# VITA-Group/SinNeRF

Hardware: AMD Instinct MI355X
Metric: rendered rays/sec (64+64 samples), lego 400x400 (higher is better)
Workload: dtype f32; 1 GPU; nerf_synthetic/lego-shaped 400x400 frame (160000 rays/GPU), N_samples=64, N_importance=64, eval render (perturb=0, noise_std=0, white_back), random-init teacher weights; points_per_ray=192, parallelism=rays sharded x1, no collective

## Files before the change

include/sinnerf_hip.h:

```cpp
#ifndef SINNERF_HIP_H
#define SINNERF_HIP_H
#include <stdint.h>
#ifdef __cplusplus
extern "C" {
#endif

#define SN_ABI_VERSION 5

#define SN_DTYPE_F32 0
#define SN_DTYPE_BF16 1
#define SN_DTYPE_BF16_STATE 2
#define SN_DTYPE_BF16X3 3
#define SN_DTYPE_F16 4
#define SN_DTYPE_CLASSIC_HEADS 0x100
#define SN_DTYPE_COMPILER_SCHEDULED 0x200
#define SN_DTYPE_EMB_BF16 0x400

#define SN_E_BADARG (-1)
#define SN_E_TOOLARGE (-2)
#define SN_E_MISSING_RNG (-3)
#define SN_E_UNSUPPORTED (-4)
#define SN_E_BADSHAPE (-5)

#define SN_FLAG_BF16_COMPILER_SCHEDULED 2
#define SN_FLAG_F32_LDS_RING 4

int sn_abi_version(void);
const char* sn_error_string(int code);

int sn_layout_xyz_slot_col(int lane_half, int slot);
int sn_layout_dir_slot_col(int lane_half, int slot);
int sn_layout_slab_k(int slab);
int sn_layout_n_slabs(void);

#define SN_N_RAW_TENSORS 24
long sn_packed_weights_bytes(int dtype);
long sn_pack_table_entries(void);
long sn_pack_table_entries_dtype(int dtype);
int sn_build_pack_table(int dtype, int32_t* table_host);
int sn_pack_weights(const float* const* raw_host_array_of_device_ptrs, const int32_t* table, long n_entries,
                    void* blob, int dtype, void* stream);
long sn_packed_weights_bytes_bwd(void);
long sn_pack_table_entries_bwd(void);
int sn_build_pack_table_bwd(int32_t* table_host);
long sn_packed_weights_bytes_bwd_bf16(void);
long sn_pack_table_entries_bwd_bf16(void);
int sn_build_pack_table_bwd_bf16(int32_t* table_host);
long sn_packed_weights_bytes_bwd_bf16x3(void);
long sn_pack_table_entries_bwd_bf16x3(void);
int sn_build_pack_table_bwd_bf16x3(int32_t* table_host);

int sn_sample_coarse(const float* rays, long n_rays, int n_samples, int use_disp, float perturb,
                     const float* perturb_rand, float* z_vals, void* stream);

int sn_mlp_forward(const void* blob, int dtype, const float* rays, const float* z_vals, long n_rays, int n_samples,
                   int sigma_only, int flags, float* out, void* stream);

int sn_mlp_forward_train(const void* blob, int dtype, const float* rays, const float* z_vals, long n_rays, int n_samples,
                         float* out, float* acts, float* emb, long slot_rows, void* stream);

int sn_mlp_forward_train_embedded(const void* blob, int dtype, const float* x, long n_rows, int ld, float* out,
                                  float* acts, long slot_rows, void* stream);

int sn_mlp_backward_chain(const void* blob_bwd, int dtype, const float* acts, const float* out_raw, const float* g_raw,
                          long n_points, long slot_rows, float* g_acts, float* g_out, void* stream);

int sn_dw_gemm(const void* tasks, int n_tasks, void* stream);

long sn_weight_grads_workspace_bytes(long slot_rows, int dtype);
int sn_weight_grads(const void* acts, const float* emb, const void* g_acts, long slot_rows, int dtype, void* workspace,
                    float* const* grads_host_array_of_device_ptrs, int accumulate, void* stream);

int sn_composite_backward(const float* raw, const float* z_vals, const float* rays, const float* noise, float noise_std,
                          long n_rays, int n_samples, int white_back, const float* g_rgb, const float* g_depth,
                          const float* g_weights, float* g_raw, void* stream);

int sn_mlp_forward_embedded(const void* blob, int dtype, const float* x, long n_rows, int ld, int sigma_only,
                            int flags, float* out, void* stream);

int sn_composite_forward(const float* raw, int has_rgb, const float* z_vals, const float* rays, const float* noise,
                         float noise_std, long n_rays, int n_samples, int white_back, float* rgb, float* depth,
                         float* weights, void* stream);

int sn_sample_pdf(const float* z_vals, const float* weights, const float* u, long n_rays, int n_samples,
                  int n_importance, float* z_fine, float* z_merged, void* stream);

int sn_sample_pdf_bins(const float* bins, const float* weights, const float* u, long n_rays, int n_bins,
                       int n_importance, float eps, float* samples, void* stream);


int sn_generate_rays(const float* c2w, int H, int W, float focal, float near, float far, int x0, int y0, int stride_x,
                     int stride_y, int patch_w, int patch_h, float* rays, void* stream);

int sn_adam_step(float* params, const float* grads, float* exp_avg, float* exp_avg_sq, long n, float lr, float beta1,
                 float beta2, float eps, float weight_decay, int step, void* stream);

long sn_render_loss_workspace_bytes(void);
int sn_render_loss(const float* rgb_coarse, const float* rgb_fine, const float* depth_coarse, const float* depth_fine,
                   const float* rgb_gt, const float* depth_gt, const unsigned char* mask, int mask_mode, long n,
                   float w_rgb, float w_depth, float* g_rgb_coarse, float* g_rgb_fine, float* g_depth_coarse,
                   float* g_depth_fine, void* workspace, float* out, void* stream);

#ifdef __cplusplus
}
#endif
#endif
```

sinnerf_amd/_lib.py:

```python
import ctypes
import os

_HERE = os.path.dirname(os.path.abspath(__file__))
LIB_PATH = os.environ.get("SINNERF_HIP_LIB") or os.path.join(_HERE, "csrc", "libsinnerf_hip.so")

SN_DTYPE_F32 = 0
SN_DTYPE_BF16 = 1
SN_DTYPE_BF16_STATE = 2
SN_DTYPE_BF16X3 = 3
SN_DTYPE_F16 = 4
SN_DTYPE_CLASSIC_HEADS = 0x100
SN_FLAG_F32_LDS_RING = 4
SN_DTYPE_COMPILER_SCHEDULED = 0x200
N_RAW_TENSORS = 24
SN_DTYPE_EMB_BF16 = 0x400
ABI_VERSION = 5

c_fp = ctypes.c_void_p
c_vp = ctypes.c_void_p
_long, _int, _float = ctypes.c_long, ctypes.c_int, ctypes.c_float

SIGNATURES = {
    "sn_abi_version": (_int, []),
    "sn_error_string": (ctypes.c_char_p, [_int]),
    "sn_layout_xyz_slot_col": (_int, [_int, _int]),
    "sn_layout_dir_slot_col": (_int, [_int, _int]),
    "sn_layout_slab_k": (_int, [_int]),
    "sn_layout_n_slabs": (_int, []),
    "sn_packed_weights_bytes": (_long, [_int]),
    "sn_pack_table_entries": (_long, []),
    "sn_pack_table_entries_dtype": (_long, [_int]),
    "sn_build_pack_table": (_int, [_int, c_vp]),
    "sn_pack_weights": (_int, [ctypes.POINTER(c_vp), c_vp, _long, c_vp, _int, c_vp]),
    "sn_packed_weights_bytes_bwd": (_long, []),
    "sn_pack_table_entries_bwd": (_long, []),
    "sn_build_pack_table_bwd": (_int, [c_vp]),
    "sn_packed_weights_bytes_bwd_bf16": (_long, []),
    "sn_pack_table_entries_bwd_bf16": (_long, []),
    "sn_build_pack_table_bwd_bf16": (_int, [c_vp]),
    "sn_packed_weights_bytes_bwd_bf16x3": (_long, []),
    "sn_pack_table_entries_bwd_bf16x3": (_long, []),
    "sn_build_pack_table_bwd_bf16x3": (_int, [c_vp]),
    "sn_sample_coarse": (_int, [c_fp, _long, _int, _int, _float, c_fp, c_fp, c_vp]),
    "sn_mlp_forward": (_int, [c_vp, _int, c_fp, c_fp, _long, _int, _int, _int, c_fp, c_vp]),
    "sn_mlp_forward_train": (_int, [c_vp, _int, c_fp, c_fp, _long, _int, c_fp, c_fp, c_fp, _long, c_vp]),
    "sn_mlp_forward_train_embedded": (_int, [c_vp, _int, c_fp, _long, _int, c_fp, c_fp, _long, c_vp]),
    "sn_mlp_backward_chain": (_int, [c_vp, _int, c_fp, c_fp, c_fp, _long, _long, c_fp, c_fp, c_vp]),
    "sn_dw_gemm": (_int, [c_vp, _int, c_vp]),
    "sn_weight_grads_workspace_bytes": (_long, [_long, _int]),
    "sn_weight_grads": (_int, [c_vp, c_fp, c_vp, _long, _int, c_vp, ctypes.POINTER(c_vp), _int, c_vp]),
    "sn_generate_rays": (_int, [c_fp, _int, _int, _float, _float, _float, _int, _int, _int, _int, _int, _int, c_fp, c_vp]),
    "sn_adam_step": (_int, [c_fp, c_fp, c_fp, c_fp, _long, _float, _float, _float, _float, _float, _int, c_vp]),
    "sn_render_loss_workspace_bytes": (_long, []),
    "sn_render_loss": (_int, [c_fp, c_fp, c_fp, c_fp, c_fp, c_fp, c_vp, _int, _long, _float, _float, c_fp, c_fp, c_fp, c_fp,
                              c_vp, c_fp, c_vp]),
    "sn_composite_backward": (_int, [c_fp, c_fp, c_fp, c_fp, _float, _long, _int, _int, c_fp, c_fp, c_fp, c_fp, c_vp]),
    "sn_mlp_forward_embedded": (_int, [c_vp, _int, c_fp, _long, _int, _int, _int, c_fp, c_vp]),
    "sn_composite_forward": (_int, [c_fp, _int, c_fp, c_fp, c_fp, _float, _long, _int, _int, c_fp, c_fp, c_fp, c_vp]),
    "sn_sample_pdf": (_int, [c_fp, c_fp, c_fp, _long, _int, _int, c_fp, c_fp, c_vp]),
    "sn_sample_pdf_bins": (_int, [c_fp, c_fp, c_fp, _long, _int, _int, _float, c_fp, c_vp]),
}


class SinnerfHipError(RuntimeError):
    pass


def _load():
    if not os.path.exists(LIB_PATH):
        raise ImportError(
            f"{LIB_PATH} not found: the HIP extension is not built. Run `python -c 'import __graft_entry__ as g; "
            "g.build()'` (or `make -C sinnerf_amd/csrc`). There is no CPU fallback for this path.")
    lib = ctypes.CDLL(LIB_PATH)
    for name, (res, args) in SIGNATURES.items():
        fn = getattr(lib, name)
        fn.restype, fn.argtypes = res, args
    if lib.sn_abi_version() != ABI_VERSION:
        raise ImportError(f"{LIB_PATH}: ABI version {lib.sn_abi_version()} != {ABI_VERSION}; rebuild the extension")
    return lib


lib = _load()


def check(code, what):
    if code != 0:
        msg = lib.sn_error_string(int(code))
        raise SinnerfHipError(f"{what} failed: [{code}] {msg.decode() if msg else '?'}")


def ptr(t):
    if t is None:
        return None
    assert t.is_contiguous(), "sinnerf_amd kernels need contiguous tensors"
    return ctypes.c_void_p(t.data_ptr())


def stream_ptr():
    import torch
    return ctypes.c_void_p(torch.cuda.current_stream().cuda_stream)
```

sinnerf_amd/autograd.py:

```python
import torch

from . import _lib
from .nerf import dtype_code


COMPILER_SCHEDULED = bool(int(__import__("os").environ.get("SINNERF_COMPILER_SCHEDULED", "0")))
EMB_BF16 = not bool(int(__import__("os").environ.get("SINNERF_EMB_FP32", "0")))


_EMB16_OK = None


def _emb16_supported():
    global _EMB16_OK
    if _EMB16_OK is None:
        _EMB16_OK = _lib.lib.sn_weight_grads_workspace_bytes(256, _lib.SN_DTYPE_BF16_STATE | _lib.SN_DTYPE_EMB_BF16) >= 0
    return _EMB16_OK


def _sched_flag():
    return _lib.SN_DTYPE_COMPILER_SCHEDULED if COMPILER_SCHEDULED else 0


def _state_code(model, acts, emb=None):
    if dtype_code(model.compute_dtype) == _lib.SN_DTYPE_BF16X3:
        return _lib.SN_DTYPE_BF16X3
    if dtype_code(model.compute_dtype) != _lib.SN_DTYPE_BF16:
        return _lib.SN_DTYPE_F32
    code = _lib.SN_DTYPE_BF16_STATE if acts.dtype == torch.bfloat16 else _lib.SN_DTYPE_BF16
    if emb is not None and emb.dtype == torch.bfloat16:
        code |= _lib.SN_DTYPE_EMB_BF16
    return code


def _sink_of(model, raws, needs):
    sink = getattr(model, "_grad_sink", None)
    if sink is None:
        return None
    for t, s_, need in zip(raws, sink, needs):
        if need and (t.grad is None or t.grad.data_ptr() != s_.data_ptr() or t.grad.shape != t.shape):
            return None
    return sink


def _weight_grads(model, acts, emb, G, needs):
    import ctypes
    dev = acts.device
    code = _state_code(model, acts, emb)
    rows = acts.shape[1]
    nbytes = _lib.lib.sn_weight_grads_workspace_bytes(rows, code)
    if nbytes < 0:
        _lib.check(int(nbytes), "sn_weight_grads_workspace_bytes")
    ws = torch.empty(int(nbytes), dtype=torch.uint8, device=dev)
    raws = model.raw_tensors()
    sink = _sink_of(model, raws, needs)
    if sink is not None:
        outs, accumulate = [s_ if need else None for s_, need in zip(sink, needs)], 1
    else:
        flat = torch.empty(sum(t.numel() for t, need in zip(raws, needs) if need), dtype=torch.float32, device=dev)
        outs, off, accumulate = [], 0, 0
        for t, need in zip(raws, needs):
            if need:
                outs.append(flat[off:off + t.numel()].view(t.shape))
                off += t.numel()
            else:
                outs.append(None)
    arr = (ctypes.c_void_p * _lib.N_RAW_TENSORS)(*[None if o is None else o.data_ptr() for o in outs])
    _lib.check(_lib.lib.sn_weight_grads(_lib.ptr(acts), _lib.ptr(emb), _lib.ptr(G), rows, code, _lib.ptr(ws), arr, accumulate,
                                        _lib.stream_ptr()), "sn_weight_grads")
    return [None] * len(outs) if sink is not None else outs


class _MLPFn(torch.autograd.Function):

    @staticmethod
    def forward(ctx, model, rays, z_vals, *params):
        embedded = z_vals is None
        n, s = (rays.shape[0], 1) if embedded else z_vals.shape
        P = n * s
        dev = rays.device
        code = dtype_code(model.compute_dtype)
        bf16 = code == _lib.SN_DTYPE_BF16
        if bf16:
            code = _lib.SN_DTYPE_BF16_STATE
        out = torch.empty((n, 4) if embedded else (n, s, 4), dtype=torch.float32, device=dev)
        tile = 256 if bf16 else 128
        rows = -(-P // tile) * tile
        acts = torch.empty((10, rows, 256), dtype=torch.bfloat16 if bf16 else torch.float32, device=dev)
        if embedded:
            emb = torch.zeros((rows, 128), dtype=torch.float32, device=dev)
            emb[:n, :63] = rays[:, :63]
            emb[:n, 64:91] = rays[:, 63:90]
            _lib.check(_lib.lib.sn_mlp_forward_train_embedded(_lib.ptr(model.packed()), model.kernel_dtype(code), _lib.ptr(rays), n, rays.shape[1],
                                                              _lib.ptr(out), _lib.ptr(acts), rows, _lib.stream_ptr()),
                       "sn_mlp_forward_train_embedded")
        else:
            emb16 = bf16 and EMB_BF16 and not COMPILER_SCHEDULED and P < 2 ** 31 - 256 and _emb16_supported()
            emb = torch.empty((rows, 128), dtype=torch.bfloat16 if emb16 else torch.float32, device=dev)
            flags = _sched_flag() | (_lib.SN_DTYPE_EMB_BF16 if emb16 else 0)
            _lib.check(_lib.lib.sn_mlp_forward_train(_lib.ptr(model.packed()), model.kernel_dtype(code) | flags, _lib.ptr(rays), _lib.ptr(z_vals), n, s,
                                                     _lib.ptr(out), _lib.ptr(acts), _lib.ptr(emb), rows, _lib.stream_ptr()),
                       "sn_mlp_forward_train")
        ctx.model = model
        ctx.n_points = P
        ctx.save_for_backward(acts, emb, out)
        return out

    @staticmethod
    def backward(ctx, g_out):
        acts, emb, out = ctx.saved_tensors
        model = ctx.model
        P, rows = ctx.n_points, acts.shape[1]
        dev = acts.device
        g_out = g_out.contiguous().float()
        G = torch.empty((10, rows, 256), dtype=acts.dtype, device=dev)
        if rows > P:
            G[:, P:].zero_()
        g_o = torch.empty((P, 4), dtype=torch.float32, device=dev)
        with torch.cuda.device(dev):
            code = dtype_code(model.compute_dtype)
            if acts.dtype == torch.bfloat16:
                code = _lib.SN_DTYPE_BF16_STATE
            _lib.check(_lib.lib.sn_mlp_backward_chain(_lib.ptr(model.packed_bwd(model.compute_dtype)), model.kernel_dtype(code) | _sched_flag(),
                                                      _lib.ptr(acts), _lib.ptr(out), _lib.ptr(g_out), P, rows, _lib.ptr(G),
                                                      _lib.ptr(g_o), _lib.stream_ptr()), "sn_mlp_backward_chain")
            needs = ctx.needs_input_grad[3:]
            grads = _weight_grads(model, acts, emb, G, needs)
        return (None, None, None, *grads)


class _CompositeFn(torch.autograd.Function):
    @staticmethod
    def forward(ctx, raw, z_vals, rays, noise, noise_std, white_back):
        n, s = z_vals.shape
        dev = rays.device
        ctx.set_materialize_grads(False)
        weights = torch.empty((n, s), dtype=torch.float32, device=dev)
        rgb = torch.empty((n, 3), dtype=torch.float32, device=dev)
        depth = torch.empty((n,), dtype=torch.float32, device=dev)
        _lib.check(_lib.lib.sn_composite_forward(_lib.ptr(raw), 1, _lib.ptr(z_vals), _lib.ptr(rays), _lib.ptr(noise),
                                                 float(noise_std), n, s, int(bool(white_back)), _lib.ptr(rgb),
                                                 _lib.ptr(depth), _lib.ptr(weights), _lib.stream_ptr()),
                   "sn_composite_forward")
        ctx.save_for_backward(raw, z_vals, rays, noise if noise is not None else torch.empty(0, device=dev))
        ctx.has_noise = noise is not None
        ctx.noise_std, ctx.white_back = float(noise_std), int(bool(white_back))
        return rgb, depth, weights

    @staticmethod
    def backward(ctx, g_rgb, g_depth, g_w):
        raw, z_vals, rays, noise = ctx.saved_tensors
        n, s = z_vals.shape
        g_raw = torch.empty((n, s, 4), dtype=torch.float32, device=raw.device)
        c = lambda t: None if t is None else t.contiguous().float()
        g_rgb, g_depth, g_w = c(g_rgb), c(g_depth), c(g_w)
        with torch.cuda.device(raw.device):
            _lib.check(_lib.lib.sn_composite_backward(_lib.ptr(raw), _lib.ptr(z_vals), _lib.ptr(rays),
                                                      _lib.ptr(noise) if ctx.has_noise else None, ctx.noise_std, n, s,
                                                      ctx.white_back, _lib.ptr(g_rgb), _lib.ptr(g_depth), _lib.ptr(g_w),
                                                      _lib.ptr(g_raw), _lib.stream_ptr()), "sn_composite_backward")
        return g_raw, None, None, None, None, None


def render_rays_autograd(models, rays, N_samples, use_disp, perturb, noise_std, N_importance, white_back, test_time,
                         detach_coarse):
    from . import rendering as R
    dev = rays.device
    n = rays.shape[0]
    stream = _lib.stream_ptr()
    for m in models:
        if dtype_code(m.compute_dtype) == _lib.SN_DTYPE_F16:
            raise NotImplementedError("sinnerf_amd: compute_dtype='fp16' is an INFERENCE arithmetic (sn_mlp_forward only); train in 'bf16' "
                                      "(same matrix rate), 'bf16x3' or 'fp32', or render under torch.no_grad()")
    perturb_rand = torch.rand((n, N_samples), device=dev) if perturb > 0 else None
    z_vals = torch.empty((n, N_samples), dtype=torch.float32, device=dev)
    _lib.check(_lib.lib.sn_sample_coarse(_lib.ptr(rays), n, N_samples, int(bool(use_disp)), float(perturb),
                                         _lib.ptr(perturb_rand), _lib.ptr(z_vals), stream), "sn_sample_coarse")
    result = {}
    coarse_grad = (not detach_coarse) and (not test_time) and any(p.requires_grad for p in models[0].parameters())
    if test_time:
        with torch.no_grad():
            raw_c = R._mlp(models[0], rays, z_vals, sigma_only=True)
    elif coarse_grad:
        raw_c = _MLPFn.apply(models[0], rays, z_vals, *models[0].raw_tensors())
    else:
        with torch.no_grad():
            raw_c = R._mlp(models[0], rays, z_vals, sigma_only=False)
    noise_c = torch.randn((n, N_samples), device=dev)
    noise_c = noise_c if noise_std != 0 else None
    if test_time:
        with torch.no_grad():
            _, _, w_c = R._composite(raw_c, False, z_vals, rays, noise_c, noise_std, white_back)
        result["opacity_coarse"] = w_c
    else:
        if coarse_grad:
            rgb_c, depth_c, w_c = _CompositeFn.apply(raw_c, z_vals, rays, noise_c, noise_std, white_back)
        else:
            with torch.no_grad():
                rgb_c, depth_c, w_c = R._composite(raw_c, True, z_vals, rays, noise_c, noise_std, white_back)
        result.update(rgb_coarse=rgb_c, depth_coarse=depth_c, opacity_coarse=w_c)
    if N_importance > 0:
        u = torch.rand((n, N_importance), device=dev) if perturb > 0 else None
        z_all = torch.empty((n, N_samples + N_importance), dtype=torch.float32, device=dev)
        _lib.check(_lib.lib.sn_sample_pdf(_lib.ptr(z_vals), _lib.ptr(w_c.detach()), _lib.ptr(u), n, N_samples,
                                          N_importance, None, _lib.ptr(z_all), stream), "sn_sample_pdf")
        if any(p.requires_grad for p in models[1].parameters()):
            raw_f = _MLPFn.apply(models[1], rays, z_all, *models[1].raw_tensors())
        else:
            with torch.no_grad():
                raw_f = R._mlp(models[1], rays, z_all, sigma_only=False)
        noise_f = torch.randn((n, N_samples + N_importance), device=dev)
        noise_f = noise_f if noise_std != 0 else None
        if raw_f.requires_grad:
            rgb_f, depth_f, w_f = _CompositeFn.apply(raw_f, z_all, rays, noise_f, noise_std, white_back)
        else:
            with torch.no_grad():
                rgb_f, depth_f, w_f = R._composite(raw_f, True, z_all, rays, noise_f, noise_std, white_back)
        result.update(rgb_fine=rgb_f, depth_fine=depth_f, opacity_fine=w_f)
    else:
        if test_time:
            raise NameError("name 'rgb_coarse' is not defined (render_rays(test_time=True) needs N_importance > 0, "
                            "as in the reference: rendering.py:331)")
        result.update(rgb_fine=result["rgb_coarse"], depth_fine=result["depth_coarse"],
                      opacity_fine=result["opacity_coarse"])
    return result


def mlp_embedded_autograd(model, x, sigma_only):
    if dtype_code(model.compute_dtype) == _lib.SN_DTYPE_F16:
        raise NotImplementedError("sinnerf_amd: compute_dtype='fp16' is an INFERENCE arithmetic; call under torch.no_grad() or train in "
                                  "'bf16' / 'bf16x3' / 'fp32'")
    if x.requires_grad:
        raise NotImplementedError("sinnerf_amd.NeRF.forward: the gradient with respect to the embedded input x is not "
                                  "implemented (parameter gradients are); detach x, or differentiate through render_rays")
    x = x.contiguous().float()
    if sigma_only:
        x = torch.cat([x, torch.zeros((x.shape[0], 27), dtype=torch.float32, device=x.device)], 1)
    with torch.cuda.device(x.device):
        out = _MLPFn.apply(model, x, None, *model.raw_tensors())
    return out[:, 3:4] if sigma_only else out
```

sinnerf_amd/csrc/sn_api.hip:

```cpp
#include <hip/hip_fp16.h>
#include "../../include/sinnerf_hip.h"
#include "sn_device.h"
#include "sn_layout.h"

extern "C" {
int sn_mlp_forward_f32_launch(const void* blob, const float* in0, const float* in1, long n_points, int s_or_ld,
                              int sigma_only, int input_mode, float* out, float* acts, float* emb,
                              long slot_rows, hipStream_t stream);
int sn_mlp_forward_f32g_launch(const void* blob, const float* in0, const float* in1, long n_points, int s_or_ld, int sigma_only,
                               int input_mode, float* out, float* acts, float* emb, long slot_rows, hipStream_t stream);
int sn_mlp_forward_f32g_classic_launch(const void* blob, const float* in0, const float* in1, long n_points, int s_or_ld, int sigma_only,
                                       int input_mode, float* out, float* acts, float* emb, long slot_rows, hipStream_t stream);
int sn_mlp_forward_f32g_store_launch(const void* blob, const float* in0, const float* in1, long n_points, int s_or_ld, int sigma_only,
                                     int input_mode, float* out, float* acts, float* emb, long slot_rows, hipStream_t stream);
int sn_mlp_forward_f32g_store_classic_launch(const void* blob, const float* in0, const float* in1, long n_points, int s_or_ld, int sigma_only,
                                             int input_mode, float* out, float* acts, float* emb, long slot_rows, hipStream_t stream);
int sn_mlp_forward_f32_classic_launch(const void* blob, const float* in0, const float* in1, long n_points, int s_or_ld,
                              int sigma_only, int input_mode, float* out, float* acts, float* emb,
                              long slot_rows, hipStream_t stream);
int sn_mlp_backward_chain_f32_launch(const void* bblob, const float* acts, const float* out_raw, const float* g_raw,
                                     long n_points, long slot_rows, float* G, float* g_out, hipStream_t stream);
int sn_mlp_backward_chain_f32_classic_launch(const void* bblob, const float* acts, const float* out_raw, const float* g_raw,
                                     long n_points, long slot_rows, float* G, float* g_out, hipStream_t stream);
int sn_mlp_backward_chain_f32g_launch(const void* bblob, const float* acts, const float* out_raw, const float* g_raw, long n_points,
                                      long slot_rows, float* G, float* g_out, hipStream_t stream);
int sn_mlp_backward_chain_f32g_classic_launch(const void* bblob, const float* acts, const float* out_raw, const float* g_raw,
                                              long n_points, long slot_rows, float* G, float* g_out, hipStream_t stream);
int sn_mlp_backward_chain_bf16_launch(const void* bblob, const float* acts, const float* out_raw, const float* g_raw,
                                      long n_points, long slot_rows, float* G, float* g_out, int state_bf16,
                                      hipStream_t stream);
int sn_mlp_backward_chain_bf16_classic_launch(const void* bblob, const float* acts, const float* out_raw, const float* g_raw,
                                      long n_points, long slot_rows, float* G, float* g_out, int state_bf16,
                                      hipStream_t stream);
int sn_mlp_backward_chain_bf16x3_launch(const void* bblob, const float* acts, const float* out_raw, const float* g_raw,
                                        long n_points, long slot_rows, float* G, float* g_out, hipStream_t stream);
int sn_mlp_backward_chain_bf16x3_t_launch(const void* bblob, const float* acts, const float* out_raw, const float* g_raw,
                                          long n_points, long slot_rows, float* G, float* g_out, hipStream_t stream);
int sn_mlp_backward_chain_bf16x3_t_classic_launch(const void* bblob, const float* acts, const float* out_raw, const float* g_raw,
                                                  long n_points, long slot_rows, float* G, float* g_out, hipStream_t stream);
int sn_mlp_backward_chain_bf16x3_classic_launch(const void* bblob, const float* acts, const float* out_raw, const float* g_raw,
                                                long n_points, long slot_rows, float* G, float* g_out, hipStream_t stream);
int sn_dw_launch(const void* tasks, int n_tasks, hipStream_t stream);
long sn_weight_grads_workspace_bytes_impl(long slot_rows, int dtype, int emb16);
int sn_weight_grads_launch(const void* acts, const float* emb, const void* G, long slot_rows, int dtype, int emb16, void* workspace,
                           float* const* grads, int accumulate, hipStream_t stream);
int sn_generate_rays_launch(const float* c2w, int H, int W, float focal, float near, float far, int x0, int y0, int sx,
                            int sy, int pw, int ph, float* rays, hipStream_t stream);
int sn_adam_step_launch(float* p, const float* g, float* m, float* v, long n, float lr, float b1, float b2, float eps,
                        float wd, int step, hipStream_t stream);
long sn_render_loss_workspace_bytes_impl();
int sn_render_loss_launch(const float* rgb_c, const float* rgb_f, const float* depth_c, const float* depth_f,
                          const float* rgb_gt, const float* depth_gt, const unsigned char* mask, int mask_mode, long n,
                          float w_rgb, float w_depth, float* g_rgb_c, float* g_rgb_f, float* g_depth_c, float* g_depth_f,
                          void* workspace, float* out, hipStream_t stream);
int sn_mlp_forward_bf16_launch(const void* blob, const float* in0, const float* in1, long n_points, int s_or_ld,
                               int sigma_only, int input_mode, float* out, float* acts, float* emb, long slot_rows,
                               int state_bf16, hipStream_t stream);
int sn_mlp_forward_bf16_classic_launch(const void* blob, const float* in0, const float* in1, long n_points, int s_or_ld,
                               int sigma_only, int input_mode, float* out, float* acts, float* emb, long slot_rows,
                               int state_bf16, hipStream_t stream);
int sn_mlp_forward_bf16_f16_launch(const void* blob, const float* in0, const float* in1, long n_points, int s_or_ld,
                               int sigma_only, int input_mode, float* out, float* acts, float* emb, long slot_rows,
                               int state_bf16, hipStream_t stream);
int sn_mlp_forward_bf16_f16_classic_launch(const void* blob, const float* in0, const float* in1, long n_points, int s_or_ld,
                               int sigma_only, int input_mode, float* out, float* acts, float* emb, long slot_rows,
                               int state_bf16, hipStream_t stream);
int sn_mlp_forward_bf16_v3_f16_launch(const void* blob, const float* rays, const float* z_vals, long n_points, int n_samples,
                                  float* out, hipStream_t stream);
int sn_mlp_forward_bf16_v3_f16_classic_launch(const void* blob, const float* rays, const float* z_vals, long n_points, int n_samples,
                                  float* out, hipStream_t stream);
int sn_mlp_forward_bf16x3_launch(const void* blob, const float* in0, const float* in1, long n_points, int s_or_ld, int sigma_only,
                                 int input_mode, float* out, float* acts, float* emb, long slot_rows, hipStream_t stream);
int sn_mlp_forward_bf16x3_classic_launch(const void* blob, const float* in0, const float* in1, long n_points, int s_or_ld,
                                         int sigma_only, int input_mode, float* out, float* acts, float* emb, long slot_rows,
                                         hipStream_t stream);
int sn_mlp_forward_bf16x3_t_launch(const void* blob, const float* rays, const float* z_vals, long n_points, int n_samples, float* out,
                                   float* acts, float* emb, long slot_rows, hipStream_t stream);
int sn_mlp_forward_bf16x3_t_classic_launch(const void* blob, const float* rays, const float* z_vals, long n_points, int n_samples, float* out,
                                           float* acts, float* emb, long slot_rows, hipStream_t stream);
int sn_mlp_forward_bf16_v3_launch(const void* blob, const float* rays, const float* z_vals, long n_points, int n_samples,
                                  float* out, hipStream_t stream);
int sn_mlp_forward_bf16_v3_classic_launch(const void* blob, const float* rays, const float* z_vals, long n_points, int n_samples,
                                  float* out, hipStream_t stream);
int sn_mlp_forward_bf16_t_launch(const void* blob, const float* rays, const float* z_vals, long n_points, int n_samples, float* out,
                                 float* acts, float* emb, long slot_rows, int emb16, hipStream_t stream);
int sn_mlp_forward_bf16_t_classic_launch(const void* blob, const float* rays, const float* z_vals, long n_points, int n_samples,
                                         float* out, float* acts, float* emb, long slot_rows, int emb16, hipStream_t stream);
int sn_mlp_backward_chain_bf16_t_launch(const void* bblob, const float* acts, const float* out_raw, const float* g_raw, long n_points,
                                        long slot_rows, float* G, float* g_out, hipStream_t stream);
int sn_mlp_backward_chain_bf16_t_classic_launch(const void* bblob, const float* acts, const float* out_raw, const float* g_raw,
                                                long n_points, long slot_rows, float* G, float* g_out, hipStream_t stream);
int sn_composite_backward_launch(const float* raw, const float* z_vals, const float* rays, const float* noise,
                                 float noise_std, long n_rays, int n_samples, int white_back, const float* g_rgb,
                                 const float* g_depth, const float* g_w, float* g_raw, hipStream_t stream);
int sn_sample_coarse_launch(const float* rays, long n_rays, int n_samples, int use_disp, float perturb,
                            const float* perturb_rand, float* z_out, hipStream_t stream);
int sn_composite_forward_launch(const float* raw, int has_rgb, const float* z_vals, const float* rays,
                                const float* noise, float noise_std, long n_rays, int n_samples, int white_back,
                                float* rgb, float* depth, float* weights, hipStream_t stream);
int sn_sample_pdf_launch(const float* z_vals, const float* weights, const float* u, long n_rays, int n_samples,
                         int n_importance, float* z_fine, float* z_merged, hipStream_t stream);
int sn_sample_pdf_bins_launch(const float* bins, const float* weights, const float* u, long n_rays, int n_bins,
                              int n_importance, float eps, float* samples, hipStream_t stream);
}

namespace {
struct RawPtrs { const float* p[snl::N_RAW]; };

__device__ __forceinline__ unsigned short f32_to_bf16_rne(float f) {
  unsigned int u = __float_as_uint(f);
  if ((u & 0x7fffffffu) > 0x7f800000u) return (unsigned short)((u >> 16) | 0x40);
  u += 0x7fffu + ((u >> 16) & 1u);
  return (unsigned short)(u >> 16);
}

__global__ void __launch_bounds__(256)
pack_kernel(RawPtrs raw, const snl::PackEntry* __restrict__ table, long n, char* __restrict__ blob, int dtype) {
  for (long i = (long)blockIdx.x * blockDim.x + threadIdx.x; i < n; i += (long)gridDim.x * blockDim.x) {
    const snl::PackEntry e = table[i];
    float v = 0.0f;
    const bool as_f32 = (e.src == -2) || (e.src >= 0 && (e.src & snl::SRC_F32_FLAG));
    if (e.src >= 0) {
      const int t = (e.src >> 20) & 0x1ff, off = e.src & 0xfffff;
      const float* src = raw.p[0];
#pragma unroll
      for (int k = 1; k < snl::N_RAW; ++k) src = (t == k) ? raw.p[k] : src;
      v = src[off];
    }
    if (dtype == snl::DT_F32 || as_f32) *reinterpret_cast<float*>(blob + e.dst) = v;
    else if (e.src >= 0 && (e.src & snl::SRC_LO_FLAG))
      *reinterpret_cast<unsigned short*>(blob + e.dst) = f32_to_bf16_rne(__fsub_rn(v, __uint_as_float((unsigned)f32_to_bf16_rne(v) << 16)));
    else if (dtype == snl::DT_F16) *reinterpret_cast<__half*>(blob + e.dst) = __float2half_rn(v);
    else *reinterpret_cast<unsigned short*>(blob + e.dst) = f32_to_bf16_rne(v);
  }
}
}

extern "C" {

int sn_abi_version(void) { return SN_ABI_VERSION; }

int sn_layout_xyz_slot_col(int h, int e) { return (h < 0 || h > 1 || e < 0 || e > 31) ? -2 : snl::xyz_slot_col(h, e); }
int sn_layout_dir_slot_col(int h, int e) { return (h < 0 || h > 1 || e < 0 || e > 15) ? -2 : snl::dir_slot_col(h, e); }
int sn_layout_slab_k(int slab) { return (slab < 0 || slab >= snl::N_SLABS) ? -2 : snl::slab_k(slab); }
int sn_layout_n_slabs(void) { return snl::N_SLABS; }

const char* sn_error_string(int code) {
  switch (code) {
    case 0: return "ok";
    case SN_E_BADARG: return "bad argument";
    case SN_E_TOOLARGE: return "problem too large for one launch";
    case SN_E_MISSING_RNG: return "perturb > 0 requires the perturb_rand tensor";
    case SN_E_UNSUPPORTED: return "unsupported configuration (dtype / samples per ray)";
    case SN_E_BADSHAPE: return "bad shape";
    default: return code > 0 ? hipGetErrorString((hipError_t)code) : "unknown error";
  }
}

long sn_packed_weights_bytes(int dtype) {
  if (dtype != SN_DTYPE_F32 && dtype != SN_DTYPE_BF16 && dtype != SN_DTYPE_BF16X3 && dtype != SN_DTYPE_F16) return SN_E_UNSUPPORTED;
  return snl::blob_bytes(dtype);
}
long sn_pack_table_entries(void) { return snl::table_entries(); }
long sn_pack_table_entries_dtype(int dtype) {
  if (dtype != SN_DTYPE_F32 && dtype != SN_DTYPE_BF16 && dtype != SN_DTYPE_BF16X3 && dtype != SN_DTYPE_F16) return SN_E_UNSUPPORTED;
  return snl::table_entries_dt(dtype);
}

int sn_build_pack_table(int dtype, int32_t* table_host) {
  if (dtype != SN_DTYPE_F32 && dtype != SN_DTYPE_BF16 && dtype != SN_DTYPE_BF16X3 && dtype != SN_DTYPE_F16) return SN_E_UNSUPPORTED;
  if (!table_host) return SN_E_BADARG;
  snl::build_pack_table(dtype, reinterpret_cast<snl::PackEntry*>(table_host));
  return 0;
}

long sn_packed_weights_bytes_bwd(void) { return snl::bblob_bytes(); }
long sn_pack_table_entries_bwd(void) { return snl::b_table_entries(); }
int sn_build_pack_table_bwd(int32_t* table_host) {
  if (!table_host) return SN_E_BADARG;
  snl::build_pack_table_bwd(reinterpret_cast<snl::PackEntry*>(table_host));
  return 0;
}

long sn_packed_weights_bytes_bwd_bf16(void) { return snl::bbblob_bytes(); }
long sn_pack_table_entries_bwd_bf16(void) { return snl::bb_table_entries(); }
int sn_build_pack_table_bwd_bf16(int32_t* table_host) {
  if (!table_host) return SN_E_BADARG;
  snl::build_pack_table_bwd_bf16(reinterpret_cast<snl::PackEntry*>(table_host));
  return 0;
}

long sn_packed_weights_bytes_bwd_bf16x3(void) { return snl::bbxblob_bytes(); }
long sn_pack_table_entries_bwd_bf16x3(void) { return snl::bbx_table_entries(); }
int sn_build_pack_table_bwd_bf16x3(int32_t* table_host) {
  if (!table_host) return SN_E_BADARG;
  snl::build_pack_table_bwd_bf16x3(reinterpret_cast<snl::PackEntry*>(table_host));
  return 0;
}

int sn_pack_weights(const float* const* raw, const int32_t* table, long n_entries, void* blob, int dtype, void* stream) {
  if (dtype != SN_DTYPE_F32 && dtype != SN_DTYPE_BF16 && dtype != SN_DTYPE_BF16X3 && dtype != SN_DTYPE_F16) return SN_E_UNSUPPORTED;
  if (!raw || !table || !blob || n_entries <= 0) return SN_E_BADARG;
  RawPtrs rp;
  for (int i = 0; i < snl::N_RAW; ++i) {
    if (!raw[i]) return SN_E_BADARG;
    rp.p[i] = raw[i];
  }
  hipLaunchKernelGGL(pack_kernel, dim3(1024), dim3(256), 0, (hipStream_t)stream, rp,
                     reinterpret_cast<const snl::PackEntry*>(table), n_entries, reinterpret_cast<char*>(blob), dtype);
  return (int)hipGetLastError();
}

int sn_sample_coarse(const float* rays, long n_rays, int n_samples, int use_disp, float perturb,
                     const float* perturb_rand, float* z_vals, void* stream) {
  if (!rays || !z_vals || n_rays < 0 || n_samples < 1) return SN_E_BADARG;
  return sn_sample_coarse_launch(rays, n_rays, n_samples, use_disp, perturb, perturb_rand, z_vals, (hipStream_t)stream);
}

#define SN_HEADS(classic, name) ((classic) ? name##_classic_launch : name##_launch)

int sn_mlp_forward(const void* blob, int dtype, const float* rays, const float* z_vals, long n_rays, int n_samples,
                   int sigma_only, int flags, float* out, void* stream) {
  if (!blob || !rays || !z_vals || !out || n_rays < 0 || n_samples < 1) return SN_E_BADARG;
  const bool classic = (dtype & SN_DTYPE_CLASSIC_HEADS) && !sigma_only;
  dtype &= ~SN_DTYPE_CLASSIC_HEADS;
  if (dtype == SN_DTYPE_BF16X3)
    return SN_HEADS(classic, sn_mlp_forward_bf16x3)(blob, rays, z_vals, n_rays * (long)n_samples, n_samples, sigma_only, 0, out,
                                                    nullptr, nullptr, 0, (hipStream_t)stream);
  if (dtype == SN_DTYPE_F16) {
    if (!sigma_only && !(flags & SN_FLAG_BF16_COMPILER_SCHEDULED))
      return (classic ? sn_mlp_forward_bf16_v3_f16_classic_launch : sn_mlp_forward_bf16_v3_f16_launch)(
          blob, rays, z_vals, n_rays * (long)n_samples, n_samples, out, (hipStream_t)stream);
    return (classic ? sn_mlp_forward_bf16_f16_classic_launch : sn_mlp_forward_bf16_f16_launch)(
        blob, rays, z_vals, n_rays * (long)n_samples, n_samples, sigma_only, 0, out, nullptr, nullptr, 0, 0, (hipStream_t)stream);
  }
  if (dtype == SN_DTYPE_BF16 && !sigma_only && !(flags & SN_FLAG_BF16_COMPILER_SCHEDULED))
    return SN_HEADS(classic, sn_mlp_forward_bf16_v3)(blob, rays, z_vals, n_rays * (long)n_samples, n_samples, out, (hipStream_t)stream);
  if (dtype == SN_DTYPE_BF16)
    return SN_HEADS(classic, sn_mlp_forward_bf16)(blob, rays, z_vals, n_rays * (long)n_samples, n_samples, sigma_only, 0, out, nullptr,
                                                  nullptr, 0, 0, (hipStream_t)stream);
  if (dtype != SN_DTYPE_F32) return SN_E_UNSUPPORTED;
  if (!(flags & SN_FLAG_F32_LDS_RING))
    return SN_HEADS(classic, sn_mlp_forward_f32g)(blob, rays, z_vals, n_rays * (long)n_samples, n_samples, sigma_only, 0, out,
                                                  nullptr, nullptr, 0, (hipStream_t)stream);
  return SN_HEADS(classic, sn_mlp_forward_f32)(blob, rays, z_vals, n_rays * (long)n_samples, n_samples, sigma_only, 0,
                                               out, nullptr, nullptr, 0, (hipStream_t)stream);
}

int sn_mlp_forward_train(const void* blob, int dtype, const float* rays, const float* z_vals, long n_rays, int n_samples,
                         float* out, float* acts, float* emb, long slot_rows, void* stream) {
  if (!blob || !rays || !z_vals || !out || !acts || !emb || n_rays < 0 || n_samples < 1) return SN_E_BADARG;
  const bool classic = dtype & SN_DTYPE_CLASSIC_HEADS;
  const bool compiler_scheduled = dtype & SN_DTYPE_COMPILER_SCHEDULED;
  const int emb16 = (dtype & SN_DTYPE_EMB_BF16) ? 1 : 0;
  dtype &= ~(SN_DTYPE_CLASSIC_HEADS | SN_DTYPE_COMPILER_SCHEDULED | SN_DTYPE_EMB_BF16);
  if (dtype != SN_DTYPE_F32 && dtype != SN_DTYPE_BF16 && dtype != SN_DTYPE_BF16_STATE && dtype != SN_DTYPE_BF16X3) return SN_E_UNSUPPORTED;
  const long n_points = n_rays * (long)n_samples;
  const long tile = (dtype == SN_DTYPE_F32 || dtype == SN_DTYPE_BF16X3) ? 128 : 256;
  if (slot_rows < (n_points + tile - 1) / tile * tile) return SN_E_BADSHAPE;
  const bool hand = dtype == SN_DTYPE_BF16_STATE && !compiler_scheduled && n_points < (1l << 31) - 256;
  if (emb16 && !hand) return SN_E_UNSUPPORTED;
  if (dtype == SN_DTYPE_BF16X3) {
    if (slot_rows % 128 != 0) return SN_E_BADSHAPE;
    if (!compiler_scheduled && n_points < (1l << 31) - 256)
      return SN_HEADS(classic, sn_mlp_forward_bf16x3_t)(blob, rays, z_vals, n_points, n_samples, out, acts, emb, slot_rows, (hipStream_t)stream);
    return SN_HEADS(classic, sn_mlp_forward_bf16x3)(blob, rays, z_vals, n_points, n_samples, 0, 0, out, acts, emb, slot_rows, (hipStream_t)stream);
  }
  if (hand)
    return SN_HEADS(classic, sn_mlp_forward_bf16_t)(blob, rays, z_vals, n_points, n_samples, out, acts, emb, slot_rows, emb16, (hipStream_t)stream);
  if (dtype != SN_DTYPE_F32)
    return SN_HEADS(classic, sn_mlp_forward_bf16)(blob, rays, z_vals, n_points, n_samples, 0, 0, out, acts, emb, slot_rows,
                                                  dtype == SN_DTYPE_BF16_STATE, (hipStream_t)stream);
  if (!compiler_scheduled)
    return SN_HEADS(classic, sn_mlp_forward_f32g_store)(blob, rays, z_vals, n_points, n_samples, 0, 0, out, acts, emb, slot_rows, (hipStream_t)stream);
  return SN_HEADS(classic, sn_mlp_forward_f32)(blob, rays, z_vals, n_points, n_samples, 0, 0, out, acts, emb, slot_rows,
                                               (hipStream_t)stream);
}

int sn_mlp_forward_train_embedded(const void* blob, int dtype, const float* x, long n_rows, int ld, float* out,
                                  float* acts, long slot_rows, void* stream) {
  if (!blob || !x || !out || !acts || n_rows < 0) return SN_E_BADARG;
  float* emb = acts;
  if (ld < 90) return SN_E_BADSHAPE;
  const bool classic = dtype & SN_DTYPE_CLASSIC_HEADS;
  dtype &= ~SN_DTYPE_CLASSIC_HEADS;
  if (dtype != SN_DTYPE_F32 && dtype != SN_DTYPE_BF16_STATE && dtype != SN_DTYPE_BF16X3) return SN_E_UNSUPPORTED;
  const long tile = (dtype == SN_DTYPE_F32 || dtype == SN_DTYPE_BF16X3) ? 128 : 256;
  if (slot_rows < (n_rows + tile - 1) / tile * tile) return SN_E_BADSHAPE;
  if (dtype == SN_DTYPE_BF16X3)
    return SN_HEADS(classic, sn_mlp_forward_bf16x3)(blob, x, nullptr, n_rows, ld, 0, 1, out, acts, emb, slot_rows, (hipStream_t)stream);
  if (dtype != SN_DTYPE_F32)
    return SN_HEADS(classic, sn_mlp_forward_bf16)(blob, x, nullptr, n_rows, ld, 0, 1, out, acts, emb, slot_rows,
                                                  dtype == SN_DTYPE_BF16_STATE, (hipStream_t)stream);
  return SN_HEADS(classic, sn_mlp_forward_f32g_store)(blob, x, nullptr, n_rows, ld, 0, 1, out, acts, emb, slot_rows, (hipStream_t)stream);
}

int sn_mlp_backward_chain(const void* blob_bwd, int dtype, const float* acts, const float* out_raw, const float* g_raw,
                          long n_points, long slot_rows, float* g_acts, float* g_out, void* stream) {
  if (!blob_bwd || !acts || !out_raw || !g_raw || !g_acts || !g_out || n_points < 0) return SN_E_BADARG;
  const bool classic = dtype & SN_DTYPE_CLASSIC_HEADS;
  const bool compiler_scheduled = dtype & SN_DTYPE_COMPILER_SCHEDULED;
  dtype &= ~(SN_DTYPE_CLASSIC_HEADS | SN_DTYPE_COMPILER_SCHEDULED);
  if (dtype != SN_DTYPE_F32 && dtype != SN_DTYPE_BF16 && dtype != SN_DTYPE_BF16_STATE && dtype != SN_DTYPE_BF16X3) return SN_E_UNSUPPORTED;
  const long tile = (dtype == SN_DTYPE_F32 || dtype == SN_DTYPE_BF16X3) ? 128 : 256;
  if (slot_rows < (n_points + tile - 1) / tile * tile) return SN_E_BADSHAPE;
  if (dtype == SN_DTYPE_BF16X3) {
    if (slot_rows % 128 != 0) return SN_E_BADSHAPE;
    if (!compiler_scheduled && n_points < (1l << 31) - 256)
      return SN_HEADS(classic, sn_mlp_backward_chain_bf16x3_t)(blob_bwd, acts, out_raw, g_raw, n_points, slot_rows, g_acts, g_out, (hipStream_t)stream);
    return SN_HEADS(classic, sn_mlp_backward_chain_bf16x3)(blob_bwd, acts, out_raw, g_raw, n_points, slot_rows, g_acts, g_out, (hipStream_t)stream);
  }
  if (dtype == SN_DTYPE_BF16_STATE && !compiler_scheduled && n_points < (1l << 31) - 256)
    return SN_HEADS(classic, sn_mlp_backward_chain_bf16_t)(blob_bwd, acts, out_raw, g_raw, n_points, slot_rows, g_acts, g_out, (hipStream_t)stream);
  if (dtype != SN_DTYPE_F32)
    return SN_HEADS(classic, sn_mlp_backward_chain_bf16)(blob_bwd, acts, out_raw, g_raw, n_points, slot_rows, g_acts, g_out,
                                                         dtype == SN_DTYPE_BF16_STATE, (hipStream_t)stream);
  if (!compiler_scheduled)
    return SN_HEADS(classic, sn_mlp_backward_chain_f32g)(blob_bwd, acts, out_raw, g_raw, n_points, slot_rows, g_acts, g_out, (hipStream_t)stream);
  return SN_HEADS(classic, sn_mlp_backward_chain_f32)(blob_bwd, acts, out_raw, g_raw, n_points, slot_rows, g_acts, g_out,
                                                      (hipStream_t)stream);
}

int sn_generate_rays(const float* c2w, int H, int W, float focal, float near, float far, int x0, int y0, int stride_x,
                     int stride_y, int patch_w, int patch_h, float* rays, void* stream) {
  if (!c2w || !rays || H < 1 || W < 1 || stride_x < 1 || stride_y < 1 || patch_w < 0 || patch_h < 0) return SN_E_BADARG;
  if (x0 < 0 || y0 < 0 || (patch_w > 0 && x0 + (patch_w - 1) * stride_x >= W) || (patch_h > 0 && y0 + (patch_h - 1) * stride_y >= H))
    return SN_E_BADSHAPE;
  return sn_generate_rays_launch(c2w, H, W, focal, near, far, x0, y0, stride_x, stride_y, patch_w, patch_h, rays,
                                 (hipStream_t)stream);
}

int sn_adam_step(float* params, const float* grads, float* exp_avg, float* exp_avg_sq, long n, float lr, float beta1,
                 float beta2, float eps, float weight_decay, int step, void* stream) {
  if (!params || !grads || !exp_avg || !exp_avg_sq || n < 0 || step < 1) return SN_E_BADARG;
  return sn_adam_step_launch(params, grads, exp_avg, exp_avg_sq, n, lr, beta1, beta2, eps, weight_decay, step,
                             (hipStream_t)stream);
}

long sn_render_loss_workspace_bytes(void) { return sn_render_loss_workspace_bytes_impl(); }

int sn_render_loss(const float* rgb_coarse, const float* rgb_fine, const float* depth_coarse, const float* depth_fine,
                   const float* rgb_gt, const float* depth_gt, const unsigned char* mask, int mask_mode, long n,
                   float w_rgb, float w_depth, float* g_rgb_coarse, float* g_rgb_fine, float* g_depth_coarse,
                   float* g_depth_fine, void* workspace, float* out, void* stream) {
  if (!workspace || !out || n < 1 || mask_mode < 0 || mask_mode > 2) return SN_E_BADARG;
  if ((mask_mode == 2 && !mask) || (mask_mode != 0 && !depth_gt)) return SN_E_BADARG;
  if ((rgb_coarse || rgb_fine) && !rgb_gt) return SN_E_BADARG;
  if ((depth_coarse || depth_fine) && !depth_gt) return SN_E_BADARG;
  return sn_render_loss_launch(rgb_coarse, rgb_fine, depth_coarse, depth_fine, rgb_gt, depth_gt, mask, mask_mode, n,
                               w_rgb, w_depth, g_rgb_coarse, g_rgb_fine, g_depth_coarse, g_depth_fine, workspace, out,
                               (hipStream_t)stream);
}

int sn_dw_gemm(const void* tasks, int n_tasks, void* stream) {
  if (!tasks || n_tasks < 0) return SN_E_BADARG;
  return sn_dw_launch(tasks, n_tasks, (hipStream_t)stream);
}

long sn_weight_grads_workspace_bytes(long slot_rows, int dtype) {
  if (slot_rows < 16 || slot_rows % 16 != 0) return SN_E_BADSHAPE;
  const int emb16 = (dtype & SN_DTYPE_EMB_BF16) ? 1 : 0;
  dtype &= ~SN_DTYPE_EMB_BF16;
  if (dtype != SN_DTYPE_F32 && dtype != SN_DTYPE_BF16 && dtype != SN_DTYPE_BF16_STATE && dtype != SN_DTYPE_BF16X3) return SN_E_UNSUPPORTED;
  if (emb16 && dtype != SN_DTYPE_BF16_STATE) return SN_E_UNSUPPORTED;
  return sn_weight_grads_workspace_bytes_impl(slot_rows, dtype, emb16);
}

int sn_weight_grads(const void* acts, const float* emb, const void* g_acts, long slot_rows, int dtype, void* workspace,
                    float* const* grads, int accumulate, void* stream) {
  if (!acts || !emb || !g_acts || !workspace || !grads) return SN_E_BADARG;
  if (slot_rows < 16 || slot_rows % 16 != 0) return SN_E_BADSHAPE;
  const int emb16 = (dtype & SN_DTYPE_EMB_BF16) ? 1 : 0;
  dtype &= ~SN_DTYPE_EMB_BF16;
  if (dtype != SN_DTYPE_F32 && dtype != SN_DTYPE_BF16 && dtype != SN_DTYPE_BF16_STATE && dtype != SN_DTYPE_BF16X3) return SN_E_UNSUPPORTED;
  if (emb16 && dtype != SN_DTYPE_BF16_STATE) return SN_E_UNSUPPORTED;
  return sn_weight_grads_launch(acts, emb, g_acts, slot_rows, dtype, emb16, workspace, grads, accumulate ? 1 : 0, (hipStream_t)stream);
}

int sn_composite_backward(const float* raw, const float* z_vals, const float* rays, const float* noise, float noise_std,
                          long n_rays, int n_samples, int white_back, const float* g_rgb, const float* g_depth,
                          const float* g_weights, float* g_raw, void* stream) {
  if (!raw || !z_vals || !rays || !g_raw || n_rays < 0 || n_samples < 1) return SN_E_BADARG;
  return sn_composite_backward_launch(raw, z_vals, rays, noise, noise_std, n_rays, n_samples, white_back, g_rgb, g_depth,
                                      g_weights, g_raw, (hipStream_t)stream);
}

int sn_mlp_forward_embedded(const void* blob, int dtype, const float* x, long n_rows, int ld, int sigma_only,
                            int flags, float* out, void* stream) {
  if (!blob || !x || !out || n_rows < 0) return SN_E_BADARG;
  if (ld < (sigma_only ? 63 : 90)) return SN_E_BADSHAPE;
  const bool classic = (dtype & SN_DTYPE_CLASSIC_HEADS) && !sigma_only;
  dtype &= ~SN_DTYPE_CLASSIC_HEADS;
  if (dtype == SN_DTYPE_BF16X3)
    return SN_HEADS(classic, sn_mlp_forward_bf16x3)(blob, x, nullptr, n_rows, ld, sigma_only, 1, out, nullptr, nullptr, 0, (hipStream_t)stream);
  if (dtype == SN_DTYPE_F16)
    return (classic ? sn_mlp_forward_bf16_f16_classic_launch : sn_mlp_forward_bf16_f16_launch)(
        blob, x, nullptr, n_rows, ld, sigma_only, 1, out, nullptr, nullptr, 0, 0, (hipStream_t)stream);
  if (dtype == SN_DTYPE_BF16)
    return SN_HEADS(classic, sn_mlp_forward_bf16)(blob, x, nullptr, n_rows, ld, sigma_only, 1, out, nullptr, nullptr, 0, 0, (hipStream_t)stream);
  if (dtype != SN_DTYPE_F32) return SN_E_UNSUPPORTED;
  if (!(flags & SN_FLAG_F32_LDS_RING))
    return SN_HEADS(classic, sn_mlp_forward_f32g)(blob, x, nullptr, n_rows, ld, sigma_only, 1, out, nullptr, nullptr, 0, (hipStream_t)stream);
  return SN_HEADS(classic, sn_mlp_forward_f32)(blob, x, nullptr, n_rows, ld, sigma_only, 1,
                                               out, nullptr, nullptr, 0, (hipStream_t)stream);
}

int sn_composite_forward(const float* raw, int has_rgb, const float* z_vals, const float* rays, const float* noise,
                         float noise_std, long n_rays, int n_samples, int white_back, float* rgb, float* depth,
                         float* weights, void* stream) {
  if (!raw || !z_vals || !rays || !weights || n_rays < 0 || n_samples < 1) return SN_E_BADARG;
  if (has_rgb && (!rgb || !depth)) return SN_E_BADARG;
  return sn_composite_forward_launch(raw, has_rgb, z_vals, rays, noise, noise_std, n_rays, n_samples, white_back, rgb,
                                     depth, weights, (hipStream_t)stream);
}

int sn_sample_pdf(const float* z_vals, const float* weights, const float* u, long n_rays, int n_samples,
                  int n_importance, float* z_fine, float* z_merged, void* stream) {
  if (!z_vals || !weights || !z_merged || n_rays < 0) return SN_E_BADARG;
  return sn_sample_pdf_launch(z_vals, weights, u, n_rays, n_samples, n_importance, z_fine, z_merged, (hipStream_t)stream);
}

int sn_sample_pdf_bins(const float* bins, const float* weights, const float* u, long n_rays, int n_bins,
                       int n_importance, float eps, float* samples, void* stream) {
  if (!bins || !weights || !samples || n_rays < 0 || !(eps > 0.0f)) return SN_E_BADARG;
  return sn_sample_pdf_bins_launch(bins, weights, u, n_rays, n_bins, n_importance, eps, samples, (hipStream_t)stream);
}

}
```

sinnerf_amd/csrc/sn_mlp_fwd_bf16_v3.hip:

```cpp
#include "sn_mlp_bf16.h"
#ifndef SN_TRUNK_INC
#define SN_TRUNK_INC "sn_bf16_trunk.inc"
#endif
#include SN_TRUNK_INC

namespace snk {

constexpr int V3_SLOT_BYTES = 20480;
constexpr int V3_SLOTS = 7;
constexpr int V3_RING_BYTES = V3_SLOTS * V3_SLOT_BYTES;
constexpr int V3_TAIL_OFF = V3_RING_BYTES;
constexpr int V3_LDS_BYTES = V3_RING_BYTES + TAIL_LDS_BYTES;

SN_DEV void v3_dma_piece(unsigned& goff, const char* blob, unsigned wv1k, int lds_off, int bump) {
  asm volatile("s_add_u32 m0, %2, %3\n\ts_nop 0\n\tglobal_load_lds_dwordx4 %0, %1\n\tv_add_u32 %0, %4, %0"
               : "+v"(goff) : "s"(blob), "s"(wv1k), "n"(lds_off), "n"(bump) : "memory", "scc");
}

template <int T, class Pending>
SN_DEV void v3_dir_slab(f32x16 (&acc)[PT], f32x16 (&accn)[PT], const char* smem, int lane, const u32x4* de,
                        const float* lds_bias, int h, unsigned& goff, const char* blob, unsigned wv1k, Pending&& pending) {
  constexpr int S = 72 + T;
  constexpr int NK = 18;
  const char* lw = smem + (S % V3_SLOTS) * V3_SLOT_BYTES + lane * 16;
  u32x4 af[4];
#pragma unroll
  for (int i = 0; i < 3; ++i) af[i] = *reinterpret_cast<const u32x4*>(lw + i * 1024);
  constexpr int TGT_SLOT = T + 1;
  constexpr int IN_FLIGHT = (T == 0) ? 11 : (T == 1) ? 7 : 3;
#pragma unroll
  for (int ks = 0; ks < NK; ++ks) {
    if (ks == 2) {
      asm volatile("s_waitcnt vmcnt(%0)" ::"n"(IN_FLIGHT) : "memory");
      __builtin_amdgcn_s_barrier();
      asm volatile("" ::: "memory");
#pragma unroll
      for (int pt = 0; pt < PT; ++pt) accn[pt] = load_bias(lds_bias, (S + 1) % snl::N_SLABS, h);
    }
    if (ks + 3 < NK) af[(ks + 3) & 3] = *reinterpret_cast<const u32x4*>(lw + (ks + 3) * 1024);
    if (ks == 2) v3_dma_piece(goff, blob, wv1k, TGT_SLOT * V3_SLOT_BYTES, 4096);
    __builtin_amdgcn_sched_barrier(0);
    const u32x4 a_cur = af[ks & 3];
#pragma unroll
    for (int pt = 0; pt < PT; ++pt) {
      if (ks == 0) mma_a<true>(acc[pt], a_cur, act_reg(0, 0, pt));
      else if (ks < 16) mma_a<false>(acc[pt], a_cur, act_reg(0, ks, pt));
      else mma_v<false>(acc[pt], a_cur, de[(ks - 16) * PT + pt]);
    }
    __builtin_amdgcn_sched_barrier(0);
    if (ks == 0) {
      pending();
      __builtin_amdgcn_sched_barrier(0);
    }
  }
}

__global__ void __launch_bounds__(256)
mlp_fwd_bf16_v3_kernel(const char* __restrict__ blob, const float* __restrict__ rays, const float* __restrict__ z_vals,
                       long P, int S, float* __restrict__ out) {
  extern __shared__ __attribute__((aligned(16))) char smem[];
  float* lds_bias = reinterpret_cast<float*>(smem + V3_TAIL_OFF);
  const float* lds_aux = lds_bias + snl::BIAS_FLOATS;
  asm volatile("" ::: "a0", "a255");

  const int tid = threadIdx.x;
  const int lane = tid & 63;
  const int wave = tid >> 6;
  const int j = lane & 31;
  const int h = lane >> 5;
  constexpr int TILE_PTS = 4 * PT * 32;
  const long n_tiles = (P + TILE_PTS - 1) / TILE_PTS;
  const unsigned wv1k = __builtin_amdgcn_readfirstlane(wave * 1024);
  const unsigned long long dma_exec_mask = 0ull;

  unsigned goff = (unsigned)(tid * 16);
  v3_dma_piece(goff, blob, wv1k, 0 * V3_SLOT_BYTES, 4096);
  v3_dma_piece(goff, blob, wv1k, 1 * V3_SLOT_BYTES, 4096);
  v3_dma_piece(goff, blob, wv1k, 2 * V3_SLOT_BYTES, 4096);
  v3_dma_piece(goff, blob, wv1k, 3 * V3_SLOT_BYTES, 4096);
  v3_dma_piece(goff, blob, wv1k, 4 * V3_SLOT_BYTES, 4096);
  {
    const float4* gb = reinterpret_cast<const float4*>(blob + snl::bias_byte_offset(snl::DT_BF16));
    float4* lb = reinterpret_cast<float4*>(lds_bias);
    for (int i = tid; i < snl::TAIL_FLOATS / 4; i += 256) lb[i] = gb[i];
  }
  asm volatile("s_waitcnt vmcnt(0)" ::: "memory");
  __syncthreads();

  const unsigned va0 = (unsigned)(lane * 16);
  const unsigned vb = (unsigned)(V3_TAIL_OFF + h * 64);
  const unsigned vs = (unsigned)(V3_TAIL_OFF + (snl::BIAS_FLOATS + snl::AUX_SIGW + h * 128) * 4);

  struct TileIn { float o[3], d[3], z; };
  auto point_of = [&](long tile, int pt) __attribute__((always_inline)) {
    const long pr = ((tile * 4 + wave) * PT + pt) * 32 + j;
    return pr < P ? pr : P - 1;
  };
  TileIn cur[PT];
  float nxt_z[PT];
  if ((long)blockIdx.x < n_tiles) {
#pragma unroll
    for (int pt = 0; pt < PT; ++pt) {
      const long pc = point_of(blockIdx.x, pt);
      nxt_z[pt] = z_vals[pc];
    }
  }

  for (long tile = blockIdx.x; tile < n_tiles; tile += gridDim.x) {
    int ht = h;
    asm volatile("" : "+v"(ht));
    u32x4 xe[4 * PT];
#pragma unroll
    for (int pt = 0; pt < PT; ++pt) {
      {
        const float* rp = rays + (point_of(tile, pt) / S) * 8;
        cur[pt].o[0] = rp[0]; cur[pt].o[1] = rp[1]; cur[pt].o[2] = rp[2];
        cur[pt].d[0] = rp[3]; cur[pt].d[1] = rp[4]; cur[pt].d[2] = rp[5];
        cur[pt].z = nxt_z[pt];
      }
      float f[32];
      const float zz = cur[pt].z;
      const float x = __fadd_rn(cur[pt].o[0], __fmul_rn(cur[pt].d[0], zz));
      const float y = __fadd_rn(cur[pt].o[1], __fmul_rn(cur[pt].d[1], zz));
      const float z = __fadd_rn(cur[pt].o[2], __fmul_rn(cur[pt].d[2], zz));
#ifdef SN_V3_NO_NONTRUNK_VALU
#pragma unroll
      for (int e = 0; e < 32; ++e) f[e] = x + (float)e * y + z;
#else
      embed_xyz_bf16(x, y, z, ht, f);
#endif
#pragma unroll
      for (int ks = 0; ks < 4; ++ks) {
        xe[ks * PT + pt] = pack8(f + 8 * ks);
        asm volatile("" : "+v"(xe[ks * PT + pt]));
      }
      __builtin_amdgcn_sched_barrier(0);
    }
    {
      const long tn = tile + gridDim.x < n_tiles ? tile + gridDim.x : tile;
#pragma unroll
      for (int pt = 0; pt < PT; ++pt) {
        const long pc = point_of(tn, pt);
        nxt_z[pt] = z_vals[pc];
      }
    }

    float sg0 = 0.0f, sg1 = 0.0f;
    asm volatile(SN_BF16_TRUNK_ASM
                 : [goff] "+v"(goff), [sg0] "+v"(sg0), [sg1] "+v"(sg1)
                 : [xe0] "v"(xe[0]), [xe1] "v"(xe[1]), [xe2] "v"(xe[2]), [xe3] "v"(xe[3]), [xe4] "v"(xe[4]), [xe5] "v"(xe[5]),
                   [xe6] "v"(xe[6]), [xe7] "v"(xe[7]), [va0] "v"(va0), [vb] "v"(vb), [vs] "v"(vs),
                   [blob] "s"(blob), [wv1k] "s"(wv1k), [em] "s"(dma_exec_mask)
                 : SN_BF16_TRUNK_CLOBBERS);

    float sigma[PT];
    sigma[0] = sg0 + __shfl_xor(sg0, 32, 64) + lds_aux[snl::AUX_HEADB];
    sigma[1] = sg1 + __shfl_xor(sg1, 32, 64) + lds_aux[snl::AUX_HEADB];

    u32x4 de[2 * PT];
#pragma unroll
    for (int pt = 0; pt < PT; ++pt) {
      float f[16];
#ifdef SN_V3_NO_NONTRUNK_VALU
#pragma unroll
      for (int e = 0; e < 16; ++e) f[e] = cur[pt].d[0] + (float)e * cur[pt].d[1];
#else
      embed_dir_bf16(cur[pt].d[0], cur[pt].d[1], cur[pt].d[2], ht, f);
#endif
      de[0 * PT + pt] = pack8(f);
      de[1 * PT + pt] = pack8(f + 8);
      asm volatile("" : "+v"(de[0 * PT + pt]), "+v"(de[1 * PT + pt]));
      __builtin_amdgcn_sched_barrier(0);
    }
    f32x2 c3[PT][3];
#pragma unroll
    for (int pt = 0; pt < PT; ++pt) c3[pt][0] = c3[pt][1] = c3[pt][2] = f32x2{0.0f, 0.0f};
    auto ssp_tile = [&](int t, const f32x16 (&r)[PT]) __attribute__((always_inline)) {
#pragma unroll
      for (int q = 0; q < 4; ++q) {
        f32x4 w[3];
#pragma unroll
        for (int c = 0; c < 3; ++c)
          w[c] = *reinterpret_cast<const f32x4*>(lds_aux + snl::AUX_RGBW + c * 128 + h * 64 + 16 * t + 4 * q);
#pragma unroll
        for (int pt = 0; pt < PT; ++pt) {
          float x[4];
#pragma unroll
          for (int i = 0; i < 4; ++i) x[i] = r[pt][4 * q + i];
          asm volatile("" : "+v"(x[0]), "+v"(x[1]), "+v"(x[2]), "+v"(x[3]), "+v"(c3[pt][0]), "+v"(c3[pt][1]), "+v"(c3[pt][2]));
          float v[4];
#ifdef SN_V3_NO_NONTRUNK_VALU
          c3[pt][0].x += x[0] + x[1]; c3[pt][1].x += x[2]; c3[pt][2].x += x[3] * w[0][0];
          (void)v;
#else
          ssp4_rgb(x, w, c3[pt], v);
#endif
        }
        __builtin_amdgcn_sched_barrier(0);
      }
    };
    f32x16 acc0[PT], acc1[PT];
#pragma unroll
    for (int pt = 0; pt < PT; ++pt) acc0[pt] = load_bias(lds_bias, 72, h);
    v3_dir_slab<0>(acc0, acc1, smem, lane, de, lds_bias, h, goff, blob, wv1k, [&]() __attribute__((always_inline)) {});
    v3_dir_slab<1>(acc1, acc0, smem, lane, de, lds_bias, h, goff, blob, wv1k, [&]() __attribute__((always_inline)) { ssp_tile(0, acc0); });
    v3_dir_slab<2>(acc0, acc1, smem, lane, de, lds_bias, h, goff, blob, wv1k, [&]() __attribute__((always_inline)) { ssp_tile(1, acc1); });
    v3_dir_slab<3>(acc1, acc0, smem, lane, de, lds_bias, h, goff, blob, wv1k, [&]() __attribute__((always_inline)) { ssp_tile(2, acc0); });
    mfma_result_fence();
    ssp_tile(3, acc1);
#pragma unroll
    for (int pt = 0; pt < PT; ++pt) {
      float o3[3];
#pragma unroll
      for (int c = 0; c < 3; ++c)
        o3[c] = rgb_activation(hsum(c3[pt][c]) + __shfl_xor(hsum(c3[pt][c]), 32, 64) + lds_aux[snl::AUX_HEADB + 1 + c]);
      const long p_raw = ((tile * 4 + wave) * PT + pt) * 32 + j;
      if (p_raw < P && h == 0) {
        float4 o;
        o.x = o3[0]; o.y = o3[1]; o.z = o3[2]; o.w = sigma[pt];
        reinterpret_cast<float4*>(out)[p_raw] = o;
      }
    }
  }
  asm volatile("s_waitcnt vmcnt(0)" ::: "memory");
}

}

extern "C" int SN_LAUNCH_NAME(sn_mlp_forward_bf16_v3)(const void* blob, const float* rays, const float* z_vals, long n_points,
                                             int n_samples, float* out, hipStream_t stream) {
  using namespace snk;
  if (n_points <= 0) return 0;
  const long tiles = (n_points + 255) / 256;
  const int n_cu = snh::cu_count();
  SN_ENSURE_DYN_LDS(mlp_fwd_bf16_v3_kernel, V3_LDS_BYTES);
  hipLaunchKernelGGL(mlp_fwd_bf16_v3_kernel, dim3((unsigned)(tiles < n_cu ? tiles : n_cu)), dim3(256), V3_LDS_BYTES, stream,
                     reinterpret_cast<const char*>(blob), rays, z_vals, n_points, n_samples, out);
  return (int)hipGetLastError();
}
```

sinnerf_amd/csrc/sn_mlp_fwd_f32g.hip:

```cpp
#include "sn_mlp_f32g.h"

namespace snk {

constexpr unsigned slab_byte_offset(int s) { return (unsigned)(snl::slab_elem_offset(s) * 4); }

template <bool SIGMA_ONLY, int INPUT_MODE, bool STORE>
__global__ void __launch_bounds__(256)
mlp_fwd_f32g_kernel(const char* __restrict__ blob, const float* __restrict__ in0, const float* __restrict__ in1, long P, int S,
                    float* __restrict__ out, float* __restrict__ acts, float* __restrict__ emb, long slot_rows) {
  constexpr int FD = STORE ? FD_STORE : FD_INFER;
  constexpr int NSTEPS = STORE ? EPI_STEPS_STORE : EPI_STEPS;
  extern __shared__ __attribute__((aligned(16))) char smem[];
  float* lds_bias = reinterpret_cast<float*>(smem);
  const float* lds_aux = lds_bias + snl::BIAS_FLOATS;

  const int tid = threadIdx.x;
  const int lane = tid & 63;
  const int wave = tid >> 6;
  const int j = lane & 31;
  const int h = lane >> 5;
  const long n_tiles = (P + 127) / 128;
  constexpr int N_USED = SIGMA_ONLY ? snl::SLAB_FIN : snl::N_SLABS;

  {
    const float4* gb = reinterpret_cast<const float4*>(blob + snl::bias_byte_offset(snl::DT_F32));
    float4* lb = reinterpret_cast<float4*>(lds_bias);
    for (int i = tid; i < snl::TAIL_FLOATS / 4; i += 256) lb[i] = gb[i];
  }
  __syncthreads();

  asm volatile("" ::: "a0", "a255");
  const rsrc_t rs = __builtin_amdgcn_make_buffer_rsrc(const_cast<char*>(blob), 0, (int)snl::blob_bytes(snl::DT_F32), 0x00020000);
  unsigned voff = lane * 16;
  asm volatile("" : "+v"(voff));
  f32x4 fr[FD];
#pragma unroll
  for (int g = 0; g < FD - 1; ++g) fr[g] = load_frag(rs, voff, g * 1024);
  f32x16 acc0 = load_bias(lds_bias, 0, h), acc1;
  char* const xp = smem + TAIL_LDS_BYTES + wave * XPOSE_WAVE_BYTES;
  const unsigned xp_w = (unsigned)(j * XPOSE_PITCH + 4 * h) * 4u;
  const unsigned xp_r = (unsigned)((lane >> 3) * XPOSE_PITCH + 4 * (lane & 7)) * 4u;
  unsigned g_off = (unsigned)((lane >> 3) * 256 + 4 * (lane & 7)) * 4u;
  constexpr int EQ = STORE ? 32 : 1024;
  unsigned epi_a = STORE ? (unsigned)(size_t)xp + xp_w : (unsigned)(size_t)(smem + TAIL_LDS_BYTES + wave * EPI_WAVE_BYTES) + lane * 16;
  asm volatile("" : "+v"(g_off));
  f32x4 rowbuf[2];
  unsigned vzero;
  asm volatile("v_mov_b32 %0, 0" : "=v"(vzero));
  asm volatile("" : "+v"(epi_a));

  for (long tile = blockIdx.x; tile < n_tiles; tile += gridDim.x) {
  const long p_wave = (tile * 4 + __builtin_amdgcn_readfirstlane(wave)) * 32;
  const long p_raw = p_wave + j;
  const bool valid = p_raw < P;
  const long p = valid ? p_raw : P - 1;

  float xe[32];
  if (INPUT_MODE == 0) {
#ifdef SN_F32G_NO_RAY_LOADS
    const float ox = 0.1f, oy = 0.2f, oz = 0.3f, dx = 0.5f, dy = 0.4f, dz = -0.7f, zz = 2.0f + 1e-6f * (float)p;
#else
    const long ray = p / S;
    const float* rp = in0 + ray * 8;
    const float ox = rp[0], oy = rp[1], oz = rp[2], dx = rp[3], dy = rp[4], dz = rp[5];
    const float zz = in1[p];
#endif
    const float x = __fadd_rn(ox, __fmul_rn(dx, zz));
    const float y = __fadd_rn(oy, __fmul_rn(dy, zz));
    const float z = __fadd_rn(oz, __fmul_rn(dz, zz));
#ifdef SN_F32G_NO_VALU_BLOCKS
#pragma unroll
    for (int e = 0; e < 32; ++e) xe[e] = x + (float)e;
#else
    embed_xyz(x, y, z, h, xe);
#endif
  } else {
    const float* row = in0 + p * (long)S;
    int hh = h;
    asm volatile("" : "+v"(hh));
#pragma unroll
    for (int e = 0; e < 32; ++e) {
      const int c0 = snl::xyz_slot_col(0, e), c1 = snl::xyz_slot_col(1, e);
      const int c = hh ? c1 : c0;
      xe[e] = (c >= 0) ? row[c < 0 ? 0 : c] : 0.0f;
    }
  }

  if (STORE && INPUT_MODE == 0) {
    int hh = h;
    asm volatile("" : "+v"(hh));
    store_emb_xyz(emb + p_raw * 128, xe, hh);
  }

  float sg = 0.0f;
  float sv[16];

  auto quad = [](const f32x16& r, int q) __attribute__((always_inline)) {
    f32x4 x;
    x[0] = r[4 * q]; x[1] = r[4 * q + 1]; x[2] = r[4 * q + 2]; x[3] = r[4 * q + 3];
    return x;
  };
  const long p_wave_c = p_wave;
  auto row_read = [&](int i) __attribute__((always_inline)) {
    return *reinterpret_cast<const f32x4*>(xp + xp_r + 8 * i * XPOSE_PITCH * 4);
  };
  auto row_store = [&](int slot, int t, int i, const f32x4& o) __attribute__((always_inline)) {
    const char* base = reinterpret_cast<const char*>(acts) + (((long)slot * slot_rows + p_wave_c + 8 * i) * 256 + 32 * t) * 4;
#ifdef SN_F32G_NO_ROW_STORES
    asm volatile("" :: "v"(o), "s"(base), "v"(g_off));
#else
    __builtin_nontemporal_store(o, reinterpret_cast<f32x4*>(const_cast<char*>(base) + g_off));
#endif
  };
  auto row_step = [&](int slot, int t, int k) __attribute__((always_inline)) {
    if (!STORE) return;
    if (k == 0) rowbuf[0] = row_read(0);
    else if (k == 1) rowbuf[1] = row_read(1);
    else if (k == 2) { row_store(slot, t, 0, rowbuf[0]); rowbuf[0] = row_read(2); }
    else if (k == 3) { row_store(slot, t, 1, rowbuf[1]); rowbuf[1] = row_read(3); }
    else if (k == 4) row_store(slot, t, 2, rowbuf[0]);
    else if (k == 5) row_store(slot, t, 3, rowbuf[1]);
  };
  f32x4 sw[4];
  auto relu_prog = [&](auto wset, auto slot_c, int t, int st, const f32x16& r) __attribute__((always_inline)) {
    constexpr int W = decltype(wset)::value;
    constexpr int slot = decltype(slot_c)::value;
    const int q = st / 6, k = st % 6;
    if (slot == 7) {
      if (st == 0) {
#pragma unroll
        for (int i = 0; i < 4; ++i) sw[i] = *reinterpret_cast<const f32x4*>(lds_aux + snl::AUX_SIGW + h * 128 + 16 * t + 4 * i);
      } else if (st == 3) {
#ifdef SN_F32G_NO_VALU_BLOCKS
#pragma unroll
        for (int i = 0; i < 16; ++i) sv[i] = r[i];
        if (false)
#endif
#pragma unroll
        for (int i = 0; i < 16; ++i) sv[i] = relu1(r[i]);
#pragma unroll
#ifndef SN_F32G_NO_VALU_BLOCKS
        for (int i = 0; i < 16; ++i) sg = __builtin_fmaf(sw[i / 4][i % 4], sv[i], sg);
#else
        for (int i = 0; i < 1; ++i) sg += sv[0];
#endif
        asm volatile("" : "+v"(sg));
      } else if (st >= 4 && st < 8) {
        f32x4 x;
        x[0] = sv[4 * (st - 4)]; x[1] = sv[4 * (st - 4) + 1]; x[2] = sv[4 * (st - 4) + 2]; x[3] = sv[4 * (st - 4) + 3];
        lds_put_quad(epi_a, EQ * (st - 4), x);
      } else if (st >= 8 && st < 12) {
        lds_get_quad_agpr(W * 128 + 16 * t + 4 * (st - 8), epi_a, EQ * (st - 8));
      } else if (st >= 24) {
        row_step(7, t, st - 24);
      }
      return;
    }
    if (st >= 24) { row_step(slot, t, st - 24); return; }
    if (k == 0) lds_put_quad(epi_a, EQ * q, quad(r, q));
#ifndef SN_F32G_NO_ATOMICS
    else if (k < 5) lds_relu_word(epi_a, EQ * q + 4 * (k - 1), vzero);
#endif
    else if (k == 5) lds_get_quad_agpr(W * 128 + 16 * t + 4 * q, epi_a, EQ * q);
  };
  auto copy_prog = [&](auto wset, auto, int t, int st, const f32x16& r) __attribute__((always_inline)) {
    constexpr int W = decltype(wset)::value;
    const int q = st / 6, k = st % 6;
    if (st >= 24) { row_step(8, t, st - 24); return; }
    if (k == 0) lds_put_quad(epi_a, EQ * q, quad(r, q));
    else if (k == 5) lds_get_quad_agpr(W * 128 + 16 * t + 4 * q, epi_a, EQ * q);
  };
  auto no_prog = [&](auto, auto, int, int, const f32x16&) __attribute__((always_inline)) {};

#define SN_C(V_) std::integral_constant<int, V_>{}
#define SN_SLABG(S_, NG0_, NG1_, S0_, S1_, BV_, PEPI_, PW_, PSLOT_, PT_)                                                  \
  do {                                                                                                                    \
    constexpr int s_nx = ((S_) + 1 == N_USED) ? 0 : (S_) + 1;                                                             \
    constexpr int g0 = (int)(slab_byte_offset(S_) / 1024), tot = (int)(slab_byte_offset(N_USED) / 1024);                  \
    if (((S_) & 1) == 0)                                                                                                  \
      slab_f32g<NG0_, NG1_, S0_, S1_, g0, tot, NSTEPS, FD>(acc0, acc1, fr, rs, voff, BV_,                                             \
          lds_bias, s_nx, h, [&](int st) __attribute__((always_inline)) { PEPI_(SN_C(PW_), SN_C(PSLOT_), PT_, st, acc1); }); \
    else                                                                                                                  \
      slab_f32g<NG0_, NG1_, S0_, S1_, g0, tot, NSTEPS, FD>(acc1, acc0, fr, rs, voff, BV_,                                             \
          lds_bias, s_nx, h, [&](int st) __attribute__((always_inline)) { PEPI_(SN_C(PW_), SN_C(PSLOT_), PT_, st, acc0); }); \
  } while (0)
#define SN_LAYERG(L_, NG0_, NG1_, S0_, S1_, EPI_, W_, PEPI_, PW_, PSLOT_)                 \
  do {                                                                                    \
    SN_SLABG(8 * (L_) + 0, NG0_, NG1_, S0_, S1_, xe, PEPI_, PW_, PSLOT_, 7);              \
    SN_SLABG(8 * (L_) + 1, NG0_, NG1_, S0_, S1_, xe, EPI_, W_, L_, 0);                    \
    SN_SLABG(8 * (L_) + 2, NG0_, NG1_, S0_, S1_, xe, EPI_, W_, L_, 1);                    \
    SN_SLABG(8 * (L_) + 3, NG0_, NG1_, S0_, S1_, xe, EPI_, W_, L_, 2);                    \
    SN_SLABG(8 * (L_) + 4, NG0_, NG1_, S0_, S1_, xe, EPI_, W_, L_, 3);                    \
    SN_SLABG(8 * (L_) + 5, NG0_, NG1_, S0_, S1_, xe, EPI_, W_, L_, 4);                    \
    SN_SLABG(8 * (L_) + 6, NG0_, NG1_, S0_, S1_, xe, EPI_, W_, L_, 5);                    \
    SN_SLABG(8 * (L_) + 7, NG0_, NG1_, S0_, S1_, xe, EPI_, W_, L_, 6);                    \
  } while (0)

  SN_LAYERG(0, 8, 0, -1, -1, relu_prog, 0, no_prog, 0, 0);
  SN_LAYERG(1, 32, 0, 0, 0, relu_prog, 1, relu_prog, 0, 0);
  SN_LAYERG(2, 32, 0, 1, 1, relu_prog, 0, relu_prog, 1, 1);
  SN_LAYERG(3, 32, 0, 0, 0, relu_prog, 1, relu_prog, 0, 2);
  SN_LAYERG(4, 8, 32, -1, 1, relu_prog, 0, relu_prog, 1, 3);
  SN_LAYERG(5, 32, 0, 0, 0, relu_prog, 1, relu_prog, 0, 4);
  SN_LAYERG(6, 32, 0, 1, 1, relu_prog, 0, relu_prog, 1, 5);
  SN_LAYERG(7, 32, 0, 0, 0, relu_prog, 1, relu_prog, 0, 6);

  if (SIGMA_ONLY) {
    mfma32_result_fence(acc1);
#pragma unroll
    for (int st = 0; st < EPI_STEPS; ++st) relu_prog(SN_C(1), SN_C(7), 7, st, acc1);
    const float sigma = sg + __shfl_xor(sg, 32, 64) + lds_aux[snl::AUX_HEADB];
    if (valid && h == 0) out[p_raw] = sigma;
    continue;
  }

  SN_LAYERG(8, 32, 0, 1, 1, copy_prog, 0, relu_prog, 1, 7);
  const float sigma = sg + __shfl_xor(sg, 32, 64) + lds_aux[snl::AUX_HEADB];

  float de[16];
  if (INPUT_MODE == 0) {
    const float* rp = in0 + (p / S) * 8;
#ifdef SN_F32G_NO_VALU_BLOCKS
#pragma unroll
    for (int e = 0; e < 16; ++e) de[e] = rp[3] + (float)e;
#else
    embed_dir(rp[3], rp[4], rp[5], h, de);
#endif
  } else {
    const float* row = in0 + p * (long)S;
    int hh = h;
    asm volatile("" : "+v"(hh));
#pragma unroll
    for (int e = 0; e < 16; ++e) {
      const int c0 = snl::dir_slot_col(0, e), c1 = snl::dir_slot_col(1, e);
      const int c = hh ? c1 : c0;
      de[e] = (c >= 0) ? row[63 + (c < 0 ? 0 : c)] : 0.0f;
    }
  }
  if (STORE && INPUT_MODE == 0) {
    int hh = h;
    asm volatile("" : "+v"(hh));
    store_emb_dir(emb + p_raw * 128 + 64, de, hh);
  }
  float c3[3] = {0.0f, 0.0f, 0.0f};
  auto ssp_slice = [&](auto, auto, int t, int st, const f32x16& r) __attribute__((always_inline)) {
    if (st >= 24) { row_step(9, t, st - 24); return; }
    if (st % 6 != 0) return;
    const int q = st / 6;
    float v[4];
#pragma unroll
#ifdef SN_F32G_NO_VALU_BLOCKS
    for (int i = 0; i < 4; ++i) v[i] = r[4 * q + i];
#else
    for (int i = 0; i < 4; ++i) v[i] = SN_NEWACT ? shifted_softplus_fast(r[4 * q + i]) : relu1(r[4 * q + i]);
#endif
#pragma unroll
#ifdef SN_F32G_NO_VALU_BLOCKS
    for (int c = 0; c < 1; ++c) c3[0] += v[0];
    if (false)
#endif
    for (int c = 0; c < 3; ++c) {
      const f32x4 w = *reinterpret_cast<const f32x4*>(lds_aux + snl::AUX_RGBW + c * 128 + h * 64 + 16 * t + 4 * q);
      c3[c] = __builtin_fmaf(w[0], v[0], c3[c]);
      c3[c] = __builtin_fmaf(w[1], v[1], c3[c]);
      c3[c] = __builtin_fmaf(w[2], v[2], c3[c]);
      c3[c] = __builtin_fmaf(w[3], v[3], c3[c]);
    }
    asm volatile("" : "+v"(c3[0]), "+v"(c3[1]), "+v"(c3[2]));
    if (STORE) {
      f32x4 o;
      o[0] = v[0]; o[1] = v[1]; o[2] = v[2]; o[3] = v[3];
      *reinterpret_cast<f32x4*>(xp + xp_w + 32 * q) = o;
    }
  };
  SN_SLABG(72, 32, 4, 0, -1, de, copy_prog, 0, 8, 7);
  SN_SLABG(73, 32, 4, 0, -1, de, ssp_slice, 0, 9, 0);
  SN_SLABG(74, 32, 4, 0, -1, de, ssp_slice, 0, 9, 1);
  SN_SLABG(75, 32, 4, 0, -1, de, ssp_slice, 0, 9, 2);
  mfma32_result_fence(acc1);
#pragma unroll
  for (int q = 0; q < 4; ++q) ssp_slice(SN_C(0), SN_C(9), 3, 6 * q, acc1);
  if (STORE) {
#pragma unroll
    for (int i = 0; i < 4; ++i) row_store(9, 3, i, row_read(i));
  }

  {
    float o3[3];
#pragma unroll
    for (int c = 0; c < 3; ++c) o3[c] = c3[c] + __shfl_xor(c3[c], 32, 64) + lds_aux[snl::AUX_HEADB + 1 + c];
    if (valid && h == 0) {
      float4 o;
      o.x = rgb_activation(o3[0]);
      o.y = rgb_activation(o3[1]);
      o.z = rgb_activation(o3[2]);
      o.w = sigma;
      reinterpret_cast<float4*>(out)[p_raw] = o;
    }
  }
  }
#undef SN_C
#undef SN_SLABG
#undef SN_LAYERG
}

}

#ifdef SN_F32G_TU_STORE
#define SN_F32G_ENTRY sn_mlp_forward_f32g_store
#else
#define SN_F32G_ENTRY sn_mlp_forward_f32g
#endif
#define SN_F32G_LAUNCH_NAME(base) SN_LAUNCH_NAME(base)
extern "C" int SN_F32G_LAUNCH_NAME(SN_F32G_ENTRY)(const void* blob, const float* in0, const float* in1, long n_points, int s_or_ld,
                                             int sigma_only, int input_mode, float* out, float* acts, float* emb, long slot_rows,
                                             hipStream_t stream) {
  using namespace snk;
  if (n_points <= 0) return 0;
  const long tiles = (n_points + 127) / 128;
  const bool store = acts != nullptr;
  if (store && (sigma_only || emb == nullptr || slot_rows < tiles * 128)) return -1;
  const int n_cu = snh::cu_count();
  dim3 grid((unsigned)(tiles < n_cu ? tiles : n_cu)), block(256);
  const size_t lds = store ? F32G_LDS_BYTES_STORE : F32G_LDS_BYTES;
  const char* b = reinterpret_cast<const char*>(blob);
#define SN_LAUNCH(SO, IM, ST)                                                                                       \
  do {                                                                                                              \
    auto kfn = mlp_fwd_f32g_kernel<SO, IM, ST>;                                                                     \
    SN_ENSURE_DYN_LDS(kfn, lds);                                                                                    \
    hipLaunchKernelGGL(kfn, grid, block, lds, stream, b, in0, in1, n_points, s_or_ld, out, acts, emb, slot_rows);   \
  } while (0)
#if defined(SN_F32G_AB)
#ifdef SN_F32G_AB_STORE
  if (!store || input_mode != 0) return -4;
  SN_LAUNCH(false, 0, true);
#else
  if (store || sigma_only || input_mode != 0) return -4;
  SN_LAUNCH(false, 0, false);
#endif
#elif defined(SN_F32G_TU_STORE)
  if (!store) return -4;
  if (input_mode == 0) SN_LAUNCH(false, 0, true); else SN_LAUNCH(false, 1, true);
#elif defined(SN_CLASSIC_HEADS)
  if (store || sigma_only) return -4;
  if (input_mode == 0) SN_LAUNCH(false, 0, false); else SN_LAUNCH(false, 1, false);
#else
  if (store) return -4;
  if (input_mode == 0) { if (sigma_only) SN_LAUNCH(true, 0, false); else SN_LAUNCH(false, 0, false); }
  else { if (sigma_only) SN_LAUNCH(true, 1, false); else SN_LAUNCH(false, 1, false); }
#endif
#undef SN_LAUNCH
  return (int)hipGetLastError();
}
```

sinnerf_amd/csrc/sn_next.hip:

```cpp
#include "sn_device.h"

namespace snx {

__global__ void __launch_bounds__(256)
generate_rays_kernel(const float* __restrict__ c2w, int H, int W, float focal, float near, float far, int x0, int y0,
                     int sx, int sy, int pw, int ph, float* __restrict__ rays) {
  const long total = (long)pw * ph;
  const float r00 = c2w[0], r01 = c2w[1], r02 = c2w[2], tx = c2w[3];
  const float r10 = c2w[4], r11 = c2w[5], r12 = c2w[6], ty = c2w[7];
  const float r20 = c2w[8], r21 = c2w[9], r22 = c2w[10], tz = c2w[11];
  const float hw = (float)W / 2.0f, hh = (float)H / 2.0f;
  for (long idx = (long)blockIdx.x * blockDim.x + threadIdx.x; idx < total; idx += (long)gridDim.x * blockDim.x) {
    const int iy = (int)(idx / pw), ix = (int)(idx - (long)iy * pw);
    const float i = (float)(x0 + ix * sx), j = (float)(y0 + iy * sy);
    const float d0 = __fdiv_rn(__fsub_rn(i, hw), focal);
    const float d1 = -__fdiv_rn(__fsub_rn(j, hh), focal);
    const float d2 = -1.0f;
    float4 lo, hi;
    lo.x = tx; lo.y = ty; lo.z = tz;
    lo.w = __fadd_rn(__fadd_rn(__fmul_rn(d0, r00), __fmul_rn(d1, r01)), __fmul_rn(d2, r02));
    hi.x = __fadd_rn(__fadd_rn(__fmul_rn(d0, r10), __fmul_rn(d1, r11)), __fmul_rn(d2, r12));
    hi.y = __fadd_rn(__fadd_rn(__fmul_rn(d0, r20), __fmul_rn(d1, r21)), __fmul_rn(d2, r22));
    hi.z = near; hi.w = far;
    float4* out = reinterpret_cast<float4*>(rays + idx * 8);
    out[0] = lo; out[1] = hi;
  }
}

__global__ void __launch_bounds__(256)
adam_kernel(float* __restrict__ p, const float* __restrict__ g, float* __restrict__ m, float* __restrict__ v, long n,
            float lr, float b1, float b2, float eps, float wd, float bc1, float bc2_sqrt) {
  const float step_size = lr / bc1;
  for (long i = (long)blockIdx.x * blockDim.x + threadIdx.x; i < n; i += (long)gridDim.x * blockDim.x) {
    float gi = g[i];
    const float pi = p[i];
    if (wd != 0.0f) gi = gi + wd * pi;
    const float mi = b1 * m[i] + (1.0f - b1) * gi;
    const float vi = b2 * v[i] + (1.0f - b2) * gi * gi;
    m[i] = mi; v[i] = vi;
    const float denom = sqrtf(vi) / bc2_sqrt + eps;
    p[i] = pi - step_size * (mi / denom);
  }
}

constexpr int LOSS_BLOCKS = 256;

SN_DEV bool depth_counted(const float* depth_gt, const unsigned char* mask, int mask_mode, long i) {
  return mask_mode == 0 ? true : (mask_mode == 1 ? depth_gt[i] > 0.0f : mask[i] != 0);
}
SN_DEV double block_sum(double v, double* sh) {
  const int lane = threadIdx.x & 63, wave = threadIdx.x >> 6;
#pragma unroll
  for (int o = 32; o > 0; o >>= 1) v += __shfl_xor(v, o, 64);
  __syncthreads();
  if (lane == 0) sh[wave] = v;
  __syncthreads();
  return ((sh[0] + sh[1]) + sh[2]) + sh[3];
}

__global__ void __launch_bounds__(256)
loss_partials_kernel(const float* __restrict__ rgb_c, const float* __restrict__ rgb_f, const float* __restrict__ depth_c,
                     const float* __restrict__ depth_f, const float* __restrict__ rgb_gt,
                     const float* __restrict__ depth_gt, const unsigned char* __restrict__ mask, int mask_mode, long n,
                     double* __restrict__ partials) {
  __shared__ double sh[4];
  double a[5] = {0, 0, 0, 0, 0};
  const long stride = (long)gridDim.x * blockDim.x, t0 = (long)blockIdx.x * blockDim.x + threadIdx.x;
  if (rgb_gt != nullptr)
    for (long i = t0; i < 3 * n; i += stride) {
      const float g = rgb_gt[i];
      if (rgb_c != nullptr) { const float d = rgb_c[i] - g; a[0] += (double)(d * d); }
      if (rgb_f != nullptr) { const float d = rgb_f[i] - g; a[1] += (double)(d * d); }
    }
  if (depth_gt != nullptr)
    for (long i = t0; i < n; i += stride) {
      if (!depth_counted(depth_gt, mask, mask_mode, i)) continue;
      const float g = depth_gt[i];
      if (depth_c != nullptr) { const float d = fabsf(depth_c[i] - g); a[2] += (double)(d < 1.0f ? 0.5f * d * d : d - 0.5f); }
      if (depth_f != nullptr) { const float d = fabsf(depth_f[i] - g); a[3] += (double)(d < 1.0f ? 0.5f * d * d : d - 0.5f); }
      a[4] += 1.0;
    }
#pragma unroll
  for (int k = 0; k < 5; ++k) {
    const double v = block_sum(a[k], sh);
    if (threadIdx.x == 0) partials[blockIdx.x * 5 + k] = v;
  }
}

__global__ void __launch_bounds__(256)
loss_finish_kernel(const float* __restrict__ rgb_c, const float* __restrict__ rgb_f, const float* __restrict__ depth_c,
                   const float* __restrict__ depth_f, const float* __restrict__ rgb_gt,
                   const float* __restrict__ depth_gt, const unsigned char* __restrict__ mask, int mask_mode, long n,
                   float w_rgb, float w_depth, const double* __restrict__ partials, int n_partials,
                   float* __restrict__ g_rgb_c, float* __restrict__ g_rgb_f, float* __restrict__ g_depth_c,
                   float* __restrict__ g_depth_f, float* __restrict__ out) {
  __shared__ double sh[4];
  double tot[5];
#pragma unroll
  for (int k = 0; k < 5; ++k) {
    const double v = (int)threadIdx.x < n_partials ? partials[threadIdx.x * 5 + k] : 0.0;
    tot[k] = block_sum(v, sh);
  }
  const double n_rgb = 3.0 * (double)n, n_d = tot[4];
  const float mse_c = rgb_c && rgb_gt ? (float)(tot[0] / n_rgb) : 0.0f, mse_f = rgb_f && rgb_gt ? (float)(tot[1] / n_rgb) : 0.0f;
  const float sl_c = depth_c && depth_gt ? (float)(tot[2] / n_d) : 0.0f, sl_f = depth_f && depth_gt ? (float)(tot[3] / n_d) : 0.0f;
  if (blockIdx.x == 0 && threadIdx.x == 0) {
    out[0] = mse_c; out[1] = mse_f; out[2] = sl_c; out[3] = sl_f;
    out[4] = w_rgb * (mse_c + mse_f) + w_depth * (sl_c + sl_f);
    out[5] = -10.0f * log10f(mse_c); out[6] = -10.0f * log10f(mse_f);
    out[7] = (float)n_d;
  }
  const float s_rgb = (float)((double)w_rgb * 2.0 / n_rgb), s_d = (float)((double)w_depth / n_d);
  const long stride = (long)gridDim.x * blockDim.x, t0 = (long)blockIdx.x * blockDim.x + threadIdx.x;
  if (rgb_gt != nullptr)
    for (long i = t0; i < 3 * n; i += stride) {
      const float g = rgb_gt[i];
      if (g_rgb_c != nullptr && rgb_c != nullptr) g_rgb_c[i] = s_rgb * (rgb_c[i] - g);
      if (g_rgb_f != nullptr && rgb_f != nullptr) g_rgb_f[i] = s_rgb * (rgb_f[i] - g);
    }
  if (depth_gt != nullptr)
    for (long i = t0; i < n; i += stride) {
      const bool on = depth_counted(depth_gt, mask, mask_mode, i);
      const float g = depth_gt[i];
      if (g_depth_c != nullptr && depth_c != nullptr) {
        const float d = depth_c[i] - g;
        g_depth_c[i] = on ? s_d * (fabsf(d) < 1.0f ? d : (d > 0.0f ? 1.0f : -1.0f)) : 0.0f;
      }
      if (g_depth_f != nullptr && depth_f != nullptr) {
        const float d = depth_f[i] - g;
        g_depth_f[i] = on ? s_d * (fabsf(d) < 1.0f ? d : (d > 0.0f ? 1.0f : -1.0f)) : 0.0f;
      }
    }
}

}

extern "C" int sn_generate_rays_launch(const float* c2w, int H, int W, float focal, float near, float far, int x0, int y0,
                                       int sx, int sy, int pw, int ph, float* rays, hipStream_t stream) {
  const long total = (long)pw * ph;
  if (total <= 0) return 0;
  long blocks = (total + 255) / 256;
  if (blocks > 4096) blocks = 4096;
  hipLaunchKernelGGL(snx::generate_rays_kernel, dim3((unsigned)blocks), dim3(256), 0, stream, c2w, H, W, focal, near, far,
                     x0, y0, sx, sy, pw, ph, rays);
  return (int)hipGetLastError();
}

extern "C" int sn_adam_step_launch(float* p, const float* g, float* m, float* v, long n, float lr, float b1, float b2,
                                   float eps, float wd, int step, hipStream_t stream) {
  if (n <= 0) return 0;
  const double bc1 = 1.0 - pow((double)b1, (double)step), bc2 = 1.0 - pow((double)b2, (double)step);
  long blocks = (n + 255) / 256;
  if (blocks > 4096) blocks = 4096;
  hipLaunchKernelGGL(snx::adam_kernel, dim3((unsigned)blocks), dim3(256), 0, stream, p, g, m, v, n, lr, b1, b2, eps, wd,
                     (float)bc1, (float)sqrt(bc2));
  return (int)hipGetLastError();
}

extern "C" long sn_render_loss_workspace_bytes_impl() { return (long)snx::LOSS_BLOCKS * 5 * sizeof(double); }
extern "C" int sn_render_loss_launch(const float* rgb_c, const float* rgb_f, const float* depth_c, const float* depth_f,
                                     const float* rgb_gt, const float* depth_gt, const unsigned char* mask, int mask_mode,
                                     long n, float w_rgb, float w_depth, float* g_rgb_c, float* g_rgb_f, float* g_depth_c,
                                     float* g_depth_f, void* workspace, float* out, hipStream_t stream) {
  using namespace snx;
  long blocks = (3 * n + 255) / 256;
  if (blocks < 1) blocks = 1;
  if (blocks > LOSS_BLOCKS) blocks = LOSS_BLOCKS;
  double* partials = reinterpret_cast<double*>(workspace);
  hipLaunchKernelGGL(loss_partials_kernel, dim3((unsigned)blocks), dim3(256), 0, stream, rgb_c, rgb_f, depth_c, depth_f,
                     rgb_gt, depth_gt, mask, mask_mode, n, partials);
  hipLaunchKernelGGL(loss_finish_kernel, dim3((unsigned)blocks), dim3(256), 0, stream, rgb_c, rgb_f, depth_c, depth_f,
                     rgb_gt, depth_gt, mask, mask_mode, n, w_rgb, w_depth, partials, (int)blocks, g_rgb_c, g_rgb_f,
                     g_depth_c, g_depth_f, out);
  return (int)hipGetLastError();
}
```

sinnerf_amd/rendering.py:

```python
import torch

from . import _lib
from .nerf import NeRF, dtype_code

__all__ = ["render_rays", "sample_pdf"]

PROFILE = None


MAX_FUSED_SAMPLES = 1024


def _is_pow2_bands(e, in_channels, n_freqs):
    fb = getattr(e, "freq_bands", None)
    if isinstance(fb, torch.Tensor):
        key = (id(fb), fb._version, fb.data_ptr(), tuple(fb.shape), str(fb.device), in_channels, n_freqs)
        if fb.device.type == "cpu" and fb.numel() <= 16:
            key += (tuple(fb.detach().reshape(-1).tolist()),)
    else:
        try:
            key = (tuple(float(v) for v in fb), in_channels, n_freqs) if fb is not None else (None, in_channels, n_freqs)
        except TypeError:
            key = (id(fb), in_channels, n_freqs)
    hit = getattr(e, "_sn_pow2_verdict", None)
    if hit is not None and hit[0] == key:
        return hit[1]
    ok = (fb is not None and getattr(e, "in_channels", None) == in_channels and getattr(e, "N_freqs", None) == n_freqs
          and len(fb) == n_freqs)
    if ok:
        host = torch.as_tensor(fb).detach().to("cpu", torch.float64)
        ok = bool(torch.equal(host, 2.0 ** torch.arange(n_freqs, dtype=torch.float64)))
    try:
        e._sn_pow2_verdict = (key, ok)
    except Exception:
        pass
    return ok


def _fused_embeddings(embeddings):
    ex, ed = embeddings[0], embeddings[1]
    return _is_pow2_bands(ex, 3, 10) and _is_pow2_bands(ed, 3, 4)


SUPPORTED = ("NeRF(D=8, W=256, in_channels_xyz=63, in_channels_dir=27, skips=[4]) with Embedding(3, 10) / Embedding(3, 4) "
             "(logscale bands 2^k) and at most %d samples per ray" % MAX_FUSED_SAMPLES)


def _check_embeddings(embeddings):
    if not _fused_embeddings(embeddings):
        raise NotImplementedError("sinnerf_amd: the HIP kernels fuse the embedding into the MLP and exist for one configuration -- "
                                  + SUPPORTED + " (what models/sinnerf.py:133-141 and eval.py:134-137 build); got other embeddings. "
                                  "There is no torch-op fallback.")


def _mlp(model, rays, z_vals, sigma_only, flags=0):
    n, s = z_vals.shape
    out = torch.empty((n, s) if sigma_only else (n, s, 4), dtype=torch.float32, device=rays.device)
    code = dtype_code(model.compute_dtype)
    blob = model.packed()
    if PROFILE is not None:
        ev0, ev1 = torch.cuda.Event(enable_timing=True), torch.cuda.Event(enable_timing=True)
        ev0.record()
    _lib.check(_lib.lib.sn_mlp_forward(_lib.ptr(blob), model.kernel_dtype(code), _lib.ptr(rays), _lib.ptr(z_vals), n, s,
                                       int(sigma_only), flags, _lib.ptr(out), _lib.stream_ptr()), "sn_mlp_forward")
    if PROFILE is not None:
        ev1.record()
        PROFILE.append((n * s, bool(sigma_only), ev0, ev1))
    return out


def _composite(raw, has_rgb, z_vals, rays, noise, noise_std, white_back):
    n, s = z_vals.shape
    dev = rays.device
    weights = torch.empty((n, s), dtype=torch.float32, device=dev)
    rgb = torch.empty((n, 3), dtype=torch.float32, device=dev) if has_rgb else None
    depth = torch.empty((n,), dtype=torch.float32, device=dev) if has_rgb else None
    _lib.check(_lib.lib.sn_composite_forward(_lib.ptr(raw), int(has_rgb), _lib.ptr(z_vals), _lib.ptr(rays),
                                             _lib.ptr(noise), float(noise_std), n, s, int(bool(white_back)),
                                             _lib.ptr(rgb), _lib.ptr(depth), _lib.ptr(weights), _lib.stream_ptr()),
               "sn_composite_forward")
    return rgb, depth, weights


def _empty_result(dev, N_samples, N_importance, test_time):
    e = lambda *shape: torch.empty(shape, dtype=torch.float32, device=dev)
    sf = N_samples + N_importance
    res = {"opacity_coarse": e(0, N_samples)}
    if not test_time:
        res.update(rgb_coarse=e(0, 3), depth_coarse=e(0))
    elif N_importance == 0:
        raise NameError("name 'rgb_coarse' is not defined (rendering.py:331)")
    res.update(rgb_fine=e(0, 3), depth_fine=e(0), opacity_fine=e(0, sf))
    return res


def _forward_core(models, rays, N_samples, use_disp, perturb, noise_std, N_importance, white_back, test_time,
                  flags=0, keep=None):
    dev = rays.device
    n = rays.shape[0]
    if n == 0:
        return _empty_result(dev, N_samples, N_importance, test_time)
    stream = _lib.stream_ptr()
    perturb_rand = None
    if perturb > 0:
        perturb_rand = torch.rand((n, N_samples), device=dev)
    z_vals = torch.empty((n, N_samples), dtype=torch.float32, device=dev)
    _lib.check(_lib.lib.sn_sample_coarse(_lib.ptr(rays), n, N_samples, int(bool(use_disp)), float(perturb),
                                         _lib.ptr(perturb_rand), _lib.ptr(z_vals), stream), "sn_sample_coarse")
    result = {}
    raw_c = _mlp(models[0], rays, z_vals, sigma_only=bool(test_time), flags=flags)
    noise_c = torch.randn((n, N_samples), device=dev)
    rgb_c, depth_c, w_c = _composite(raw_c, not test_time, z_vals, rays, noise_c if noise_std != 0 else None,
                                     noise_std, white_back)
    if test_time:
        result["opacity_coarse"] = w_c
    else:
        result.update(rgb_coarse=rgb_c, depth_coarse=depth_c, opacity_coarse=w_c)
    if keep is not None:
        keep.update(z_coarse=z_vals, raw_coarse=raw_c, noise_coarse=noise_c if noise_std != 0 else None)
    if N_importance > 0:
        u = torch.rand((n, N_importance), device=dev) if perturb > 0 else None
        z_all = torch.empty((n, N_samples + N_importance), dtype=torch.float32, device=dev)
        _lib.check(_lib.lib.sn_sample_pdf(_lib.ptr(z_vals), _lib.ptr(w_c), _lib.ptr(u), n, N_samples, N_importance,
                                          None, _lib.ptr(z_all), stream), "sn_sample_pdf")
        raw_f = _mlp(models[1], rays, z_all, sigma_only=False, flags=flags)
        noise_f = torch.randn((n, N_samples + N_importance), device=dev)
        rgb_f, depth_f, w_f = _composite(raw_f, True, z_all, rays, noise_f if noise_std != 0 else None, noise_std,
                                         white_back)
        result.update(rgb_fine=rgb_f, depth_fine=depth_f, opacity_fine=w_f)
        if keep is not None:
            keep.update(z_fine=z_all, raw_fine=raw_f, noise_fine=noise_f if noise_std != 0 else None)
    else:
        if test_time:
            raise NameError("name 'rgb_coarse' is not defined (render_rays(test_time=True) needs N_importance > 0, "
                            "as in the reference: rendering.py:331)")
        result.update(rgb_fine=rgb_c, depth_fine=depth_c, opacity_fine=w_c)
    return result


def render_rays(models,
                embeddings,
                rays,
                N_samples=64,
                use_disp=False,
                perturb=0,
                noise_std=1,
                N_importance=0,
                chunk=1024 * 32,
                white_back=False,
                test_time=False,
                detach_coarse=False,
                noisy_coarse=True,
                ):
    if not isinstance(rays, torch.Tensor) or not rays.is_cuda:
        raise RuntimeError("sinnerf_amd.render_rays: rays must be a CUDA/ROCm tensor (there is no CPU fallback)")
    if rays.dim() != 2 or rays.shape[1] != 8:
        raise RuntimeError(f"rays must have shape (N_rays, 8), got {tuple(rays.shape)}")
    for m in models:
        if not isinstance(m, NeRF):
            raise TypeError("sinnerf_amd.render_rays needs sinnerf_amd.NeRF models (state_dict-compatible with "
                            "the reference NeRF; load reference weights with load_state_dict)")
    if N_importance > 0 and len(models) < 2:
        raise IndexError("list index out of range")
    rays = rays.contiguous().float()
    _check_embeddings(embeddings)
    if N_samples + N_importance > MAX_FUSED_SAMPLES:
        raise NotImplementedError("sinnerf_amd.render_rays: %d + %d samples per ray; the per-ray kernels (compositor, importance "
                                  "sampler, merge) hold at most %d in one wave.  Supported: %s"
                                  % (N_samples, N_importance, MAX_FUSED_SAMPLES, SUPPORTED))
    needs_grad = torch.is_grad_enabled() and any(p.requires_grad for m in models for p in m.parameters())
    with torch.cuda.device(rays.device):
        if needs_grad and rays.shape[0] > 0:
            from .autograd import render_rays_autograd
            return render_rays_autograd(models, rays, N_samples, use_disp, perturb, noise_std, N_importance,
                                        white_back, test_time, detach_coarse)
        with torch.no_grad():
            return _forward_core(models, rays, N_samples, use_disp, perturb, noise_std, N_importance, white_back,
                                 test_time)


@torch.no_grad()
def eval_points(points, models, embeddings):
    _check_embeddings(embeddings)
    if points.dim() != 2 or points.shape[1] != 3:
        raise RuntimeError(f"eval_points: points must be (B, 3), got {tuple(points.shape)}")
    if points.shape[0] == 0:
        return torch.empty((0, 1), dtype=torch.float32, device=points.device)
    return models[-1](embeddings[0](points.float()), sigma_only=True)


def sample_pdf(bins, weights, N_importance, det=False, eps=1e-5):
    if not bins.is_cuda:
        raise RuntimeError("sinnerf_amd.sample_pdf: CUDA/ROCm tensors only (no CPU fallback)")
    if not eps > 0:
        raise ValueError("sample_pdf: eps must be positive")
    n, m = weights.shape
    bins = bins.contiguous().float()
    weights = weights.detach().contiguous().float()
    with torch.cuda.device(bins.device):
        u = None if det else torch.rand((n, N_importance), device=bins.device)
        out = torch.empty((n, N_importance), dtype=torch.float32, device=bins.device)
        _lib.check(_lib.lib.sn_sample_pdf_bins(_lib.ptr(bins), _lib.ptr(weights), _lib.ptr(u), n, m, N_importance, float(eps),
                                               _lib.ptr(out), _lib.stream_ptr()), "sn_sample_pdf_bins")
    return out
```

Baseline: 661,700 rays/s.

## Precompute per-ray direction embeddings once and reuse across coarse and fine MLPs

Adds a small kernel that computes the view-direction positional embedding once per ray (split into two lane halves) and stores it in a table. The fused MLP kernels can now load this embedding, prefetched during an early pipeline stage, instead of recomputing sin/cos for every sample point. The table is built once per render call and shared between the coarse and fine passes. The cost is an extra kernel launch, a table allocation, and extra global memory reads in exchange for less VALU work per point.

```diff
diff --git a/include/sinnerf_hip.h b/include/sinnerf_hip.h
--- a/include/sinnerf_hip.h
+++ b/include/sinnerf_hip.h
@@ -56,8 +56,15 @@
 int sn_mlp_forward(const void* blob, int dtype, const float* rays, const float* z_vals, long n_rays, int n_samples,
                    int sigma_only, int flags, float* out, void* stream);
 
+int sn_embed_dirs(const float* rays, long n_rays, int dtype, void* table, void* stream);
+int sn_mlp_forward_dirs(const void* blob, int dtype, const float* rays, const float* z_vals, long n_rays, int n_samples,
+                        int sigma_only, int flags, const void* dir_table, float* out, void* stream);
+
 int sn_mlp_forward_train(const void* blob, int dtype, const float* rays, const float* z_vals, long n_rays, int n_samples,
                          float* out, float* acts, float* emb, long slot_rows, void* stream);
+
+int sn_mlp_forward_train_dirs(const void* blob, int dtype, const float* rays, const float* z_vals, long n_rays, int n_samples,
+                              const void* dir_table, float* out, float* acts, float* emb, long slot_rows, void* stream);
 
 int sn_mlp_forward_train_embedded(const void* blob, int dtype, const float* x, long n_rows, int ld, float* out,
                                   float* acts, long slot_rows, void* stream);
diff --git a/sinnerf_amd/_lib.py b/sinnerf_amd/_lib.py
--- a/sinnerf_amd/_lib.py
+++ b/sinnerf_amd/_lib.py
@@ -43,7 +43,10 @@
     "sn_build_pack_table_bwd_bf16x3": (_int, [c_vp]),
     "sn_sample_coarse": (_int, [c_fp, _long, _int, _int, _float, c_fp, c_fp, c_vp]),
     "sn_mlp_forward": (_int, [c_vp, _int, c_fp, c_fp, _long, _int, _int, _int, c_fp, c_vp]),
+    "sn_embed_dirs": (_int, [c_fp, _long, _int, c_vp, c_vp]),
+    "sn_mlp_forward_dirs": (_int, [c_vp, _int, c_fp, c_fp, _long, _int, _int, _int, c_vp, c_fp, c_vp]),
     "sn_mlp_forward_train": (_int, [c_vp, _int, c_fp, c_fp, _long, _int, c_fp, c_fp, c_fp, _long, c_vp]),
+    "sn_mlp_forward_train_dirs": (_int, [c_vp, _int, c_fp, c_fp, _long, _int, c_vp, c_fp, c_fp, c_fp, _long, c_vp]),
     "sn_mlp_forward_train_embedded": (_int, [c_vp, _int, c_fp, _long, _int, c_fp, c_fp, _long, c_vp]),
     "sn_mlp_backward_chain": (_int, [c_vp, _int, c_fp, c_fp, c_fp, _long, _long, c_fp, c_fp, c_vp]),
     "sn_dw_gemm": (_int, [c_vp, _int, c_vp]),
diff --git a/sinnerf_amd/autograd.py b/sinnerf_amd/autograd.py
--- a/sinnerf_amd/autograd.py
+++ b/sinnerf_amd/autograd.py
@@ -9,6 +9,7 @@
 
 
 _EMB16_OK = None
+_ACTIVE_TABLES = None
 
 
 def _emb16_supported():
@@ -98,8 +99,10 @@
             emb16 = bf16 and EMB_BF16 and not COMPILER_SCHEDULED and P < 2 ** 31 - 256 and _emb16_supported()
             emb = torch.empty((rows, 128), dtype=torch.bfloat16 if emb16 else torch.float32, device=dev)
             flags = _sched_flag() | (_lib.SN_DTYPE_EMB_BF16 if emb16 else 0)
-            _lib.check(_lib.lib.sn_mlp_forward_train(_lib.ptr(model.packed()), model.kernel_dtype(code) | flags, _lib.ptr(rays), _lib.ptr(z_vals), n, s,
-                                                     _lib.ptr(out), _lib.ptr(acts), _lib.ptr(emb), rows, _lib.stream_ptr()),
+            tables = _ACTIVE_TABLES
+            dir_table = tables.get(code) if tables is not None and tables.rays is rays and code == _lib.SN_DTYPE_F32 else None
+            _lib.check(_lib.lib.sn_mlp_forward_train_dirs(_lib.ptr(model.packed()), model.kernel_dtype(code) | flags, _lib.ptr(rays), _lib.ptr(z_vals), n, s,
+                                                          _lib.ptr(dir_table), _lib.ptr(out), _lib.ptr(acts), _lib.ptr(emb), rows, _lib.stream_ptr()),
                        "sn_mlp_forward_train")
         ctx.model = model
         ctx.n_points = P
@@ -165,6 +168,18 @@
 def render_rays_autograd(models, rays, N_samples, use_disp, perturb, noise_std, N_importance, white_back, test_time,
                          detach_coarse):
     from . import rendering as R
+    global _ACTIVE_TABLES
+    tables = _ACTIVE_TABLES = R._DirTables(rays)
+    try:
+        return _render_rays_autograd(models, rays, N_samples, use_disp, perturb, noise_std, N_importance, white_back, test_time,
+                                     detach_coarse, tables)
+    finally:
+        _ACTIVE_TABLES = None
+
+
+def _render_rays_autograd(models, rays, N_samples, use_disp, perturb, noise_std, N_importance, white_back, test_time,
+                          detach_coarse, tables):
+    from . import rendering as R
     dev = rays.device
     n = rays.shape[0]
     stream = _lib.stream_ptr()
@@ -180,12 +195,12 @@
     coarse_grad = (not detach_coarse) and (not test_time) and any(p.requires_grad for p in models[0].parameters())
     if test_time:
         with torch.no_grad():
-            raw_c = R._mlp(models[0], rays, z_vals, sigma_only=True)
+            raw_c = R._mlp(models[0], rays, z_vals, sigma_only=True, tables=tables)
     elif coarse_grad:
         raw_c = _MLPFn.apply(models[0], rays, z_vals, *models[0].raw_tensors())
     else:
         with torch.no_grad():
-            raw_c = R._mlp(models[0], rays, z_vals, sigma_only=False)
+            raw_c = R._mlp(models[0], rays, z_vals, sigma_only=False, tables=tables)
     noise_c = torch.randn((n, N_samples), device=dev)
     noise_c = noise_c if noise_std != 0 else None
     if test_time:
@@ -208,7 +223,7 @@
             raw_f = _MLPFn.apply(models[1], rays, z_all, *models[1].raw_tensors())
         else:
             with torch.no_grad():
-                raw_f = R._mlp(models[1], rays, z_all, sigma_only=False)
+                raw_f = R._mlp(models[1], rays, z_all, sigma_only=False, tables=tables)
         noise_f = torch.randn((n, N_samples + N_importance), device=dev)
         noise_f = noise_f if noise_std != 0 else None
         if raw_f.requires_grad:
diff --git a/sinnerf_amd/csrc/sn_api.hip b/sinnerf_amd/csrc/sn_api.hip
--- a/sinnerf_amd/csrc/sn_api.hip
+++ b/sinnerf_amd/csrc/sn_api.hip
@@ -8,13 +8,13 @@
                               int sigma_only, int input_mode, float* out, float* acts, float* emb,
                               long slot_rows, hipStream_t stream);
 int sn_mlp_forward_f32g_launch(const void* blob, const float* in0, const float* in1, long n_points, int s_or_ld, int sigma_only,
-                               int input_mode, float* out, float* acts, float* emb, long slot_rows, hipStream_t stream);
+                               int input_mode, float* out, float* acts, float* emb, long slot_rows, const float* dir_table, hipStream_t stream);
 int sn_mlp_forward_f32g_classic_launch(const void* blob, const float* in0, const float* in1, long n_points, int s_or_ld, int sigma_only,
-                                       int input_mode, float* out, float* acts, float* emb, long slot_rows, hipStream_t stream);
+                                       int input_mode, float* out, float* acts, float* emb, long slot_rows, const float* dir_table, hipStream_t stream);
 int sn_mlp_forward_f32g_store_launch(const void* blob, const float* in0, const float* in1, long n_points, int s_or_ld, int sigma_only,
-                                     int input_mode, float* out, float* acts, float* emb, long slot_rows, hipStream_t stream);
+                                     int input_mode, float* out, float* acts, float* emb, long slot_rows, const float* dir_table, hipStream_t stream);
 int sn_mlp_forward_f32g_store_classic_launch(const void* blob, const float* in0, const float* in1, long n_points, int s_or_ld, int sigma_only,
-                                             int input_mode, float* out, float* acts, float* emb, long slot_rows, hipStream_t stream);
+                                             int input_mode, float* out, float* acts, float* emb, long slot_rows, const float* dir_table, hipStream_t stream);
 int sn_mlp_forward_f32_classic_launch(const void* blob, const float* in0, const float* in1, long n_points, int s_or_ld,
                               int sigma_only, int input_mode, float* out, float* acts, float* emb,
                               long slot_rows, hipStream_t stream);
@@ -66,9 +66,9 @@
                                int sigma_only, int input_mode, float* out, float* acts, float* emb, long slot_rows,
                                int state_bf16, hipStream_t stream);
 int sn_mlp_forward_bf16_v3_f16_launch(const void* blob, const float* rays, const float* z_vals, long n_points, int n_samples,
-                                  float* out, hipStream_t stream);
+                                  float* out, const void* dir_table, hipStream_t stream);
 int sn_mlp_forward_bf16_v3_f16_classic_launch(const void* blob, const float* rays, const float* z_vals, long n_points, int n_samples,
-                                  float* out, hipStream_t stream);
+                                  float* out, const void* dir_table, hipStream_t stream);
 int sn_mlp_forward_bf16x3_launch(const void* blob, const float* in0, const float* in1, long n_points, int s_or_ld, int sigma_only,
                                  int input_mode, float* out, float* acts, float* emb, long slot_rows, hipStream_t stream);
 int sn_mlp_forward_bf16x3_classic_launch(const void* blob, const float* in0, const float* in1, long n_points, int s_or_ld,
@@ -79,9 +79,9 @@
 int sn_mlp_forward_bf16x3_t_classic_launch(const void* blob, const float* rays, const float* z_vals, long n_points, int n_samples, float* out,
                                            float* acts, float* emb, long slot_rows, hipStream_t stream);
 int sn_mlp_forward_bf16_v3_launch(const void* blob, const float* rays, const float* z_vals, long n_points, int n_samples,
-                                  float* out, hipStream_t stream);
+                                  float* out, const void* dir_table, hipStream_t stream);
 int sn_mlp_forward_bf16_v3_classic_launch(const void* blob, const float* rays, const float* z_vals, long n_points, int n_samples,
-                                  float* out, hipStream_t stream);
+                                  float* out, const void* dir_table, hipStream_t stream);
 int sn_mlp_forward_bf16_t_launch(const void* blob, const float* rays, const float* z_vals, long n_points, int n_samples, float* out,
                                  float* acts, float* emb, long slot_rows, int emb16, hipStream_t stream);
 int sn_mlp_forward_bf16_t_classic_launch(const void* blob, const float* rays, const float* z_vals, long n_points, int n_samples,
@@ -90,6 +90,9 @@
                                         long slot_rows, float* G, float* g_out, hipStream_t stream);
 int sn_mlp_backward_chain_bf16_t_classic_launch(const void* bblob, const float* acts, const float* out_raw, const float* g_raw,
                                                 long n_points, long slot_rows, float* G, float* g_out, hipStream_t stream);
+int sn_embed_dirs_f32_launch(const float* rays, long n_rays, float* table, hipStream_t stream);
+int sn_embed_dirs_16_launch(const float* rays, long n_rays, void* table, hipStream_t stream);
+int sn_embed_dirs_16_f16_launch(const float* rays, long n_rays, void* table, hipStream_t stream);
 int sn_composite_backward_launch(const float* raw, const float* z_vals, const float* rays, const float* noise,
                                  float noise_std, long n_rays, int n_samples, int white_back, const float* g_rgb,
                                  const float* g_depth, const float* g_w, float* g_raw, hipStream_t stream);
@@ -219,8 +222,22 @@
 
 #define SN_HEADS(classic, name) ((classic) ? name##_classic_launch : name##_launch)
 
+int sn_embed_dirs(const float* rays, long n_rays, int dtype, void* table, void* stream) {
+  if (n_rays < 0 || (n_rays > 0 && (!rays || !table))) return SN_E_BADARG;
+  dtype &= ~SN_DTYPE_CLASSIC_HEADS;
+  if (dtype != SN_DTYPE_F32 && dtype != SN_DTYPE_BF16 && dtype != SN_DTYPE_F16) return SN_E_UNSUPPORTED;
+  if (n_rays == 0) return 0;
+  if (dtype == SN_DTYPE_F32) return sn_embed_dirs_f32_launch(rays, n_rays, reinterpret_cast<float*>(table), (hipStream_t)stream);
+  return (dtype == SN_DTYPE_F16 ? sn_embed_dirs_16_f16_launch : sn_embed_dirs_16_launch)(rays, n_rays, table, (hipStream_t)stream);
+}
+
 int sn_mlp_forward(const void* blob, int dtype, const float* rays, const float* z_vals, long n_rays, int n_samples,
                    int sigma_only, int flags, float* out, void* stream) {
+  return sn_mlp_forward_dirs(blob, dtype, rays, z_vals, n_rays, n_samples, sigma_only, flags, nullptr, out, stream);
+}
+
+int sn_mlp_forward_dirs(const void* blob, int dtype, const float* rays, const float* z_vals, long n_rays, int n_samples,
+                        int sigma_only, int flags, const void* dir_table, float* out, void* stream) {
   if (!blob || !rays || !z_vals || !out || n_rays < 0 || n_samples < 1) return SN_E_BADARG;
   const bool classic = (dtype & SN_DTYPE_CLASSIC_HEADS) && !sigma_only;
   dtype &= ~SN_DTYPE_CLASSIC_HEADS;
@@ -230,25 +247,30 @@
   if (dtype == SN_DTYPE_F16) {
     if (!sigma_only && !(flags & SN_FLAG_BF16_COMPILER_SCHEDULED))
       return (classic ? sn_mlp_forward_bf16_v3_f16_classic_launch : sn_mlp_forward_bf16_v3_f16_launch)(
-          blob, rays, z_vals, n_rays * (long)n_samples, n_samples, out, (hipStream_t)stream);
+          blob, rays, z_vals, n_rays * (long)n_samples, n_samples, out, dir_table, (hipStream_t)stream);
     return (classic ? sn_mlp_forward_bf16_f16_classic_launch : sn_mlp_forward_bf16_f16_launch)(
         blob, rays, z_vals, n_rays * (long)n_samples, n_samples, sigma_only, 0, out, nullptr, nullptr, 0, 0, (hipStream_t)stream);
   }
   if (dtype == SN_DTYPE_BF16 && !sigma_only && !(flags & SN_FLAG_BF16_COMPILER_SCHEDULED))
-    return SN_HEADS(classic, sn_mlp_forward_bf16_v3)(blob, rays, z_vals, n_rays * (long)n_samples, n_samples, out, (hipStream_t)stream);
+    return SN_HEADS(classic, sn_mlp_forward_bf16_v3)(blob, rays, z_vals, n_rays * (long)n_samples, n_samples, out, dir_table, (hipStream_t)stream);
   if (dtype == SN_DTYPE_BF16)
     return SN_HEADS(classic, sn_mlp_forward_bf16)(blob, rays, z_vals, n_rays * (long)n_samples, n_samples, sigma_only, 0, out, nullptr,
                                                   nullptr, 0, 0, (hipStream_t)stream);
   if (dtype != SN_DTYPE_F32) return SN_E_UNSUPPORTED;
   if (!(flags & SN_FLAG_F32_LDS_RING))
     return SN_HEADS(classic, sn_mlp_forward_f32g)(blob, rays, z_vals, n_rays * (long)n_samples, n_samples, sigma_only, 0, out,
-                                                  nullptr, nullptr, 0, (hipStream_t)stream);
+                                                  nullptr, nullptr, 0, reinterpret_cast<const float*>(dir_table), (hipStream_t)stream);
   return SN_HEADS(classic, sn_mlp_forward_f32)(blob, rays, z_vals, n_rays * (long)n_samples, n_samples, sigma_only, 0,
                                                out, nullptr, nullptr, 0, (hipStream_t)stream);
 }
 
 int sn_mlp_forward_train(const void* blob, int dtype, const float* rays, const float* z_vals, long n_rays, int n_samples,
                          float* out, float* acts, float* emb, long slot_rows, void* stream) {
+  return sn_mlp_forward_train_dirs(blob, dtype, rays, z_vals, n_rays, n_samples, nullptr, out, acts, emb, slot_rows, stream);
+}
+
+int sn_mlp_forward_train_dirs(const void* blob, int dtype, const float* rays, const float* z_vals, long n_rays, int n_samples,
+                              const void* dir_table, float* out, float* acts, float* emb, long slot_rows, void* stream) {
   if (!blob || !rays || !z_vals || !out || !acts || !emb || n_rays < 0 || n_samples < 1) return SN_E_BADARG;
   const bool classic = dtype & SN_DTYPE_CLASSIC_HEADS;
   const bool compiler_scheduled = dtype & SN_DTYPE_COMPILER_SCHEDULED;
@@ -272,7 +294,8 @@
     return SN_HEADS(classic, sn_mlp_forward_bf16)(blob, rays, z_vals, n_points, n_samples, 0, 0, out, acts, emb, slot_rows,
                                                   dtype == SN_DTYPE_BF16_STATE, (hipStream_t)stream);
   if (!compiler_scheduled)
-    return SN_HEADS(classic, sn_mlp_forward_f32g_store)(blob, rays, z_vals, n_points, n_samples, 0, 0, out, acts, emb, slot_rows, (hipStream_t)stream);
+    return SN_HEADS(classic, sn_mlp_forward_f32g_store)(blob, rays, z_vals, n_points, n_samples, 0, 0, out, acts, emb, slot_rows,
+                                                        reinterpret_cast<const float*>(dir_table), (hipStream_t)stream);
   return SN_HEADS(classic, sn_mlp_forward_f32)(blob, rays, z_vals, n_points, n_samples, 0, 0, out, acts, emb, slot_rows,
                                                (hipStream_t)stream);
 }
@@ -292,7 +315,7 @@
   if (dtype != SN_DTYPE_F32)
     return SN_HEADS(classic, sn_mlp_forward_bf16)(blob, x, nullptr, n_rows, ld, 0, 1, out, acts, emb, slot_rows,
                                                   dtype == SN_DTYPE_BF16_STATE, (hipStream_t)stream);
-  return SN_HEADS(classic, sn_mlp_forward_f32g_store)(blob, x, nullptr, n_rows, ld, 0, 1, out, acts, emb, slot_rows, (hipStream_t)stream);
+  return SN_HEADS(classic, sn_mlp_forward_f32g_store)(blob, x, nullptr, n_rows, ld, 0, 1, out, acts, emb, slot_rows, nullptr, (hipStream_t)stream);
 }
 
 int sn_mlp_backward_chain(const void* blob_bwd, int dtype, const float* acts, const float* out_raw, const float* g_raw,
@@ -400,7 +423,7 @@
     return SN_HEADS(classic, sn_mlp_forward_bf16)(blob, x, nullptr, n_rows, ld, sigma_only, 1, out, nullptr, nullptr, 0, 0, (hipStream_t)stream);
   if (dtype != SN_DTYPE_F32) return SN_E_UNSUPPORTED;
   if (!(flags & SN_FLAG_F32_LDS_RING))
-    return SN_HEADS(classic, sn_mlp_forward_f32g)(blob, x, nullptr, n_rows, ld, sigma_only, 1, out, nullptr, nullptr, 0, (hipStream_t)stream);
+    return SN_HEADS(classic, sn_mlp_forward_f32g)(blob, x, nullptr, n_rows, ld, sigma_only, 1, out, nullptr, nullptr, 0, nullptr, (hipStream_t)stream);
   return SN_HEADS(classic, sn_mlp_forward_f32)(blob, x, nullptr, n_rows, ld, sigma_only, 1,
                                                out, nullptr, nullptr, 0, (hipStream_t)stream);
 }
diff --git a/sinnerf_amd/csrc/sn_mlp_fwd_bf16_v3.hip b/sinnerf_amd/csrc/sn_mlp_fwd_bf16_v3.hip
--- a/sinnerf_amd/csrc/sn_mlp_fwd_bf16_v3.hip
+++ b/sinnerf_amd/csrc/sn_mlp_fwd_bf16_v3.hip
@@ -56,8 +56,19 @@
 }
 
 __global__ void __launch_bounds__(256)
+embed_dirs_16_kernel(const float* __restrict__ rays, long n_rays, u32x4* __restrict__ table) {
+  for (long i = (long)blockIdx.x * 256 + threadIdx.x; i < 2 * n_rays; i += (long)gridDim.x * 256) {
+    const float* rp = rays + (i >> 1) * 8;
+    float f[16];
+    embed_dir_bf16(rp[3], rp[4], rp[5], (int)(i & 1), f);
+    table[2 * i] = pack8(f);
+    table[2 * i + 1] = pack8(f + 8);
+  }
+}
+
+__global__ void __launch_bounds__(256)
 mlp_fwd_bf16_v3_kernel(const char* __restrict__ blob, const float* __restrict__ rays, const float* __restrict__ z_vals,
-                       long P, int S, float* __restrict__ out) {
+                       long P, int S, float* __restrict__ out, const u32x4* __restrict__ dtab) {
   extern __shared__ __attribute__((aligned(16))) char smem[];
   float* lds_bias = reinterpret_cast<float*>(smem + V3_TAIL_OFF);
   const float* lds_aux = lds_bias + snl::BIAS_FLOATS;
@@ -110,10 +121,16 @@
     int ht = h;
     asm volatile("" : "+v"(ht));
     u32x4 xe[4 * PT];
+    u32x4 de[2 * PT];
 #pragma unroll
     for (int pt = 0; pt < PT; ++pt) {
       {
-        const float* rp = rays + (point_of(tile, pt) / S) * 8;
+        const long ray = point_of(tile, pt) / S;
+        const float* rp = rays + ray * 8;
+        if (dtab) {
+          de[0 * PT + pt] = dtab[ray * 4 + 2 * h];
+          de[1 * PT + pt] = dtab[ray * 4 + 2 * h + 1];
+        }
         cur[pt].o[0] = rp[0]; cur[pt].o[1] = rp[1]; cur[pt].o[2] = rp[2];
         cur[pt].d[0] = rp[3]; cur[pt].d[1] = rp[4]; cur[pt].d[2] = rp[5];
         cur[pt].z = nxt_z[pt];
@@ -135,6 +152,10 @@
         asm volatile("" : "+v"(xe[ks * PT + pt]));
       }
       __builtin_amdgcn_sched_barrier(0);
+    }
+    if (dtab) {
+#pragma unroll
+      for (int i = 0; i < 2 * PT; ++i) asm volatile("" : "+v"(de[i]));
     }
     {
       const long tn = tile + gridDim.x < n_tiles ? tile + gridDim.x : tile;
@@ -157,7 +178,7 @@
     sigma[0] = sg0 + __shfl_xor(sg0, 32, 64) + lds_aux[snl::AUX_HEADB];
     sigma[1] = sg1 + __shfl_xor(sg1, 32, 64) + lds_aux[snl::AUX_HEADB];
 
-    u32x4 de[2 * PT];
+    if (!dtab) {
 #pragma unroll
     for (int pt = 0; pt < PT; ++pt) {
       float f[16];
@@ -171,6 +192,7 @@
       de[1 * PT + pt] = pack8(f + 8);
       asm volatile("" : "+v"(de[0 * PT + pt]), "+v"(de[1 * PT + pt]));
       __builtin_amdgcn_sched_barrier(0);
+    }
     }
     f32x2 c3[PT][3];
 #pragma unroll
@@ -228,13 +250,24 @@
 }
 
 extern "C" int SN_LAUNCH_NAME(sn_mlp_forward_bf16_v3)(const void* blob, const float* rays, const float* z_vals, long n_points,
-                                             int n_samples, float* out, hipStream_t stream) {
+                                             int n_samples, float* out, const void* dir_table, hipStream_t stream) {
   using namespace snk;
   if (n_points <= 0) return 0;
   const long tiles = (n_points + 255) / 256;
   const int n_cu = snh::cu_count();
   SN_ENSURE_DYN_LDS(mlp_fwd_bf16_v3_kernel, V3_LDS_BYTES);
   hipLaunchKernelGGL(mlp_fwd_bf16_v3_kernel, dim3((unsigned)(tiles < n_cu ? tiles : n_cu)), dim3(256), V3_LDS_BYTES, stream,
-                     reinterpret_cast<const char*>(blob), rays, z_vals, n_points, n_samples, out);
+                     reinterpret_cast<const char*>(blob), rays, z_vals, n_points, n_samples, out,
+                     reinterpret_cast<const u32x4*>(dir_table));
   return (int)hipGetLastError();
 }
+
+#ifndef SN_CLASSIC_HEADS
+extern "C" int SN_LAUNCH_NAME(sn_embed_dirs_16)(const float* rays, long n_rays, void* table, hipStream_t stream) {
+  if (n_rays <= 0) return 0;
+  const long blocks = (2 * n_rays + 255) / 256;
+  hipLaunchKernelGGL(snk::embed_dirs_16_kernel, dim3((unsigned)(blocks < 4096 ? blocks : 4096)), dim3(256), 0, stream, rays, n_rays,
+                     reinterpret_cast<snk::u32x4*>(table));
+  return (int)hipGetLastError();
+}
+#endif
diff --git a/sinnerf_amd/csrc/sn_mlp_fwd_f32g.hip b/sinnerf_amd/csrc/sn_mlp_fwd_f32g.hip
--- a/sinnerf_amd/csrc/sn_mlp_fwd_f32g.hip
+++ b/sinnerf_amd/csrc/sn_mlp_fwd_f32g.hip
@@ -7,7 +7,8 @@
 template <bool SIGMA_ONLY, int INPUT_MODE, bool STORE>
 __global__ void __launch_bounds__(256)
 mlp_fwd_f32g_kernel(const char* __restrict__ blob, const float* __restrict__ in0, const float* __restrict__ in1, long P, int S,
-                    float* __restrict__ out, float* __restrict__ acts, float* __restrict__ emb, long slot_rows) {
+                    float* __restrict__ out, float* __restrict__ acts, float* __restrict__ emb, long slot_rows,
+                    const float* __restrict__ dtab) {
   constexpr int FD = STORE ? FD_STORE : FD_INFER;
   constexpr int NSTEPS = STORE ? EPI_STEPS_STORE : EPI_STEPS;
   extern __shared__ __attribute__((aligned(16))) char smem[];
@@ -48,6 +49,9 @@
   unsigned vzero;
   asm volatile("v_mov_b32 %0, 0" : "=v"(vzero));
   asm volatile("" : "+v"(epi_a));
+  const bool p32 = P < (1l << 31);
+  const bool ray_uniform = INPUT_MODE == 0 && p32 && (S & 31) == 0;
+  const bool has_dtab = __builtin_amdgcn_readfirstlane(dtab != nullptr ? 1 : 0) != 0;
 
   for (long tile = blockIdx.x; tile < n_tiles; tile += gridDim.x) {
   const long p_wave = (tile * 4 + __builtin_amdgcn_readfirstlane(wave)) * 32;
@@ -56,13 +60,24 @@
   const long p = valid ? p_raw : P - 1;
 
   float xe[32];
+  const float* dsrc = nullptr;
   if (INPUT_MODE == 0) {
 #ifdef SN_F32G_NO_RAY_LOADS
     const float ox = 0.1f, oy = 0.2f, oz = 0.3f, dx = 0.5f, dy = 0.4f, dz = -0.7f, zz = 2.0f + 1e-6f * (float)p;
 #else
-    const long ray = p / S;
-    const float* rp = in0 + ray * 8;
-    const float ox = rp[0], oy = rp[1], oz = rp[2], dx = rp[3], dy = rp[4], dz = rp[5];
+    float ox, oy, oz, dx, dy, dz;
+    if (ray_uniform) {
+      const unsigned pw = (unsigned)p_wave < (unsigned)P ? (unsigned)p_wave : (unsigned)P - 32u;
+      const long ray = (long)__builtin_amdgcn_readfirstlane((int)(pw / (unsigned)S));
+      const float* rp = in0 + ray * 8;
+      ox = rp[0]; oy = rp[1]; oz = rp[2]; dx = rp[3]; dy = rp[4]; dz = rp[5];
+      dsrc = dtab ? dtab + ray * 32 + h * 16 : rp + 3;
+    } else {
+      const long ray = p32 ? (long)((unsigned)p / (unsigned)S) : p / S;
+      const float* rp = in0 + ray * 8;
+      ox = rp[0]; oy = rp[1]; oz = rp[2]; dx = rp[3]; dy = rp[4]; dz = rp[5];
+      dsrc = dtab ? dtab + ray * 32 + h * 16 : rp + 3;
+    }
     const float zz = in1[p];
 #endif
     const float x = __fadd_rn(ox, __fmul_rn(dx, zz));
@@ -121,6 +136,7 @@
     else if (k == 4) row_store(slot, t, 2, rowbuf[0]);
     else if (k == 5) row_store(slot, t, 3, rowbuf[1]);
   };
+  f32x4 dq[4];
   f32x4 sw[4];
   auto relu_prog = [&](auto wset, auto slot_c, int t, int st, const f32x16& r) __attribute__((always_inline)) {
     constexpr int W = decltype(wset)::value;
@@ -151,6 +167,8 @@
         lds_put_quad(epi_a, EQ * (st - 4), x);
       } else if (st >= 8 && st < 12) {
         lds_get_quad_agpr(W * 128 + 16 * t + 4 * (st - 8), epi_a, EQ * (st - 8));
+      } else if (!SIGMA_ONLY && INPUT_MODE == 0 && t == 0 && st >= 12 && st < 16) {
+        if (has_dtab) dq[st - 12] = *reinterpret_cast<const f32x4*>(dsrc + 4 * (st - 12));
       } else if (st >= 24) {
         row_step(7, t, st - 24);
       }
@@ -219,12 +237,20 @@
 
   float de[16];
   if (INPUT_MODE == 0) {
-    const float* rp = in0 + (p / S) * 8;
-#ifdef SN_F32G_NO_VALU_BLOCKS
-#pragma unroll
-    for (int e = 0; e < 16; ++e) de[e] = rp[3] + (float)e;
-#else
-    embed_dir(rp[3], rp[4], rp[5], h, de);
+#if defined(SN_F32G_NO_RAY_LOADS)
+    embed_dir(0.5f, 0.4f, -0.7f, h, de);
+#elif defined(SN_F32G_NO_VALU_BLOCKS)
+#pragma unroll
+    for (int e = 0; e < 16; ++e) de[e] = dsrc[0] + (float)e;
+#else
+    if (!has_dtab) {
+      float t[16];
+      embed_dir(dsrc[0], dsrc[1], dsrc[2], h, t);
+#pragma unroll
+      for (int e = 0; e < 16; ++e) dq[e / 4][e % 4] = t[e];
+    }
+#pragma unroll
+    for (int e = 0; e < 16; ++e) de[e] = dq[e / 4][e % 4];
 #endif
   } else {
     const float* row = in0 + p * (long)S;
@@ -314,7 +340,7 @@
 #define SN_F32G_LAUNCH_NAME(base) SN_LAUNCH_NAME(base)
 extern "C" int SN_F32G_LAUNCH_NAME(SN_F32G_ENTRY)(const void* blob, const float* in0, const float* in1, long n_points, int s_or_ld,
                                              int sigma_only, int input_mode, float* out, float* acts, float* emb, long slot_rows,
-                                             hipStream_t stream) {
+                                             const float* dir_table, hipStream_t stream) {
   using namespace snk;
   if (n_points <= 0) return 0;
   const long tiles = (n_points + 127) / 128;
@@ -324,11 +350,12 @@
   dim3 grid((unsigned)(tiles < n_cu ? tiles : n_cu)), block(256);
   const size_t lds = store ? F32G_LDS_BYTES_STORE : F32G_LDS_BYTES;
   const char* b = reinterpret_cast<const char*>(blob);
+  const float* dtab = (input_mode == 0 && !sigma_only) ? dir_table : nullptr;
 #define SN_LAUNCH(SO, IM, ST)                                                                                       \
   do {                                                                                                              \
     auto kfn = mlp_fwd_f32g_kernel<SO, IM, ST>;                                                                     \
     SN_ENSURE_DYN_LDS(kfn, lds);                                                                                    \
-    hipLaunchKernelGGL(kfn, grid, block, lds, stream, b, in0, in1, n_points, s_or_ld, out, acts, emb, slot_rows);   \
+    hipLaunchKernelGGL(kfn, grid, block, lds, stream, b, in0, in1, n_points, s_or_ld, out, acts, emb, slot_rows, dtab); \
   } while (0)
 #if defined(SN_F32G_AB)
 #ifdef SN_F32G_AB_STORE
diff --git a/sinnerf_amd/csrc/sn_next.hip b/sinnerf_amd/csrc/sn_next.hip
--- a/sinnerf_amd/csrc/sn_next.hip
+++ b/sinnerf_amd/csrc/sn_next.hip
@@ -1,4 +1,29 @@
-#include "sn_device.h"
+#include "sn_mlp_common.h"
+
+namespace snk {
+__global__ void __launch_bounds__(256)
+embed_dirs_f32_kernel(const float* __restrict__ rays, long n_rays, float* __restrict__ table) {
+  for (long i = (long)blockIdx.x * 256 + threadIdx.x; i < 2 * n_rays; i += (long)gridDim.x * 256) {
+    const float* rp = rays + (i >> 1) * 8;
+    float de[16];
+    embed_dir(rp[3], rp[4], rp[5], (int)(i & 1), de);
+    f32x4* o = reinterpret_cast<f32x4*>(table + i * 16);
+#pragma unroll
+    for (int q = 0; q < 4; ++q) {
+      f32x4 v;
+      v[0] = de[4 * q]; v[1] = de[4 * q + 1]; v[2] = de[4 * q + 2]; v[3] = de[4 * q + 3];
+      o[q] = v;
+    }
+  }
+}
+}
+
+extern "C" int sn_embed_dirs_f32_launch(const float* rays, long n_rays, float* table, hipStream_t stream) {
+  if (n_rays <= 0) return 0;
+  const long blocks = (2 * n_rays + 255) / 256;
+  hipLaunchKernelGGL(snk::embed_dirs_f32_kernel, dim3((unsigned)(blocks < 4096 ? blocks : 4096)), dim3(256), 0, stream, rays, n_rays, table);
+  return (int)hipGetLastError();
+}
 
 namespace snx {
 
diff --git a/sinnerf_amd/rendering.py b/sinnerf_amd/rendering.py
--- a/sinnerf_amd/rendering.py
+++ b/sinnerf_amd/rendering.py
@@ -1,3 +1,5 @@
+import os
+
 import torch
 
 from . import _lib
@@ -6,6 +8,27 @@
 __all__ = ["render_rays", "sample_pdf"]
 
 PROFILE = None
+
+
+DIR_TABLE = bool(int(os.environ.get("SINNERF_DIR_TABLE", "1")))
+
+
+class _DirTables:
+
+    def __init__(self, rays):
+        self.rays = rays
+        self.tables = {}
+
+    def get(self, code, sigma_only=False):
+        if not DIR_TABLE or sigma_only or code not in (_lib.SN_DTYPE_F32, _lib.SN_DTYPE_BF16, _lib.SN_DTYPE_F16):
+            return None
+        t = self.tables.get(code)
+        if t is None:
+            n = self.rays.shape[0]
+            t = torch.empty((n, 32 if code == _lib.SN_DTYPE_F32 else 16), dtype=torch.float32, device=self.rays.device)
+            _lib.check(_lib.lib.sn_embed_dirs(_lib.ptr(self.rays), n, code, _lib.ptr(t), _lib.stream_ptr()), "sn_embed_dirs")
+            self.tables[code] = t
+        return t
 
 
 MAX_FUSED_SAMPLES = 1024
@@ -53,16 +76,18 @@
                                   "There is no torch-op fallback.")
 
 
-def _mlp(model, rays, z_vals, sigma_only, flags=0):
+def _mlp(model, rays, z_vals, sigma_only, flags=0, tables=None):
     n, s = z_vals.shape
     out = torch.empty((n, s) if sigma_only else (n, s, 4), dtype=torch.float32, device=rays.device)
     code = dtype_code(model.compute_dtype)
     blob = model.packed()
+    dir_table = tables.get(code, sigma_only) if tables is not None and tables.rays is rays else None
     if PROFILE is not None:
         ev0, ev1 = torch.cuda.Event(enable_timing=True), torch.cuda.Event(enable_timing=True)
         ev0.record()
-    _lib.check(_lib.lib.sn_mlp_forward(_lib.ptr(blob), model.kernel_dtype(code), _lib.ptr(rays), _lib.ptr(z_vals), n, s,
-                                       int(sigma_only), flags, _lib.ptr(out), _lib.stream_ptr()), "sn_mlp_forward")
+    _lib.check(_lib.lib.sn_mlp_forward_dirs(_lib.ptr(blob), model.kernel_dtype(code), _lib.ptr(rays), _lib.ptr(z_vals), n, s,
+                                            int(sigma_only), flags, _lib.ptr(dir_table), _lib.ptr(out), _lib.stream_ptr()),
+               "sn_mlp_forward")
     if PROFILE is not None:
         ev1.record()
         PROFILE.append((n * s, bool(sigma_only), ev0, ev1))
@@ -108,7 +133,10 @@
     _lib.check(_lib.lib.sn_sample_coarse(_lib.ptr(rays), n, N_samples, int(bool(use_disp)), float(perturb),
                                          _lib.ptr(perturb_rand), _lib.ptr(z_vals), stream), "sn_sample_coarse")
     result = {}
-    raw_c = _mlp(models[0], rays, z_vals, sigma_only=bool(test_time), flags=flags)
+    tables = _DirTables(rays)
+    if N_importance > 0:
+        tables.get(dtype_code(models[1].compute_dtype))
+    raw_c = _mlp(models[0], rays, z_vals, sigma_only=bool(test_time), flags=flags, tables=tables)
     noise_c = torch.randn((n, N_samples), device=dev)
     rgb_c, depth_c, w_c = _composite(raw_c, not test_time, z_vals, rays, noise_c if noise_std != 0 else None,
                                      noise_std, white_back)
@@ -123,7 +151,7 @@
         z_all = torch.empty((n, N_samples + N_importance), dtype=torch.float32, device=dev)
         _lib.check(_lib.lib.sn_sample_pdf(_lib.ptr(z_vals), _lib.ptr(w_c), _lib.ptr(u), n, N_samples, N_importance,
                                           None, _lib.ptr(z_all), stream), "sn_sample_pdf")
-        raw_f = _mlp(models[1], rays, z_all, sigma_only=False, flags=flags)
+        raw_f = _mlp(models[1], rays, z_all, sigma_only=False, flags=flags, tables=tables)
         noise_f = torch.randn((n, N_samples + N_importance), device=dev)
         rgb_f, depth_f, w_f = _composite(raw_f, True, z_all, rays, noise_f if noise_std != 0 else None, noise_std,
                                          white_back)
```

After: 660,500 rays/s. No clear change (-0.2%).
